# IRMVLab/EfficientLO-Net

Measured on AMD Instinct MI355X. Metric: frame-pairs/sec (KITTI 64x1800 range image), higher is better.
Workload: dtype f32 (1x1 convolutions as 3 fp16-MFMA products of hi/lo-split fp32 operands, fp32 accumulate)

## Files before the change

efficientlo-net_amd/_lib.py:

```python
import ctypes
import os

import torch

_PKG = os.path.dirname(os.path.abspath(__file__))
LIB_PATH = os.environ.get("ELO_LIB_PATH") or os.path.join(
    _PKG, "libelo_hip_f32.so" if os.environ.get("ELO_DENSE_F32", "0") == "1" else "libelo_hip.so")

_vp = ctypes.c_void_p


class GroupArgs(ctypes.Structure):
    _fields_ = [("batch", ctypes.c_int), ("H", ctypes.c_int), ("W", ctypes.c_int),
                ("H2", ctypes.c_int), ("W2", ctypes.c_int), ("npoints", ctypes.c_int),
                ("kernel_h", ctypes.c_int), ("kernel_w", ctypes.c_int), ("K", ctypes.c_int),
                ("flag_copy", ctypes.c_int), ("distance", ctypes.c_float),
                ("stride_h", ctypes.c_int), ("stride_w", ctypes.c_int),
                ("xyz1", _vp), ("xyz2", _vp), ("idx_n2", _vp), ("random_hw", _vp),
                ("selected_bhw_idx", _vp), ("valid_idx", _vp), ("valid_in_dis_idx", _vp),
                ("selected_mask", _vp)]


def _struct(name, fields):
    return type(name, (ctypes.Structure,), {"_fields_": fields, "__doc__": "struct %s (include/elo.h)." % name})


_i, _f = ctypes.c_int, ctypes.c_float
GroupConcatArgs = _struct("elo_group_concat_args", [
    ("batch", _i), ("npoints", _i), ("K", _i), ("H2", _i), ("W2", _i), ("C", _i),
    ("centre_xyz", _vp), ("src_xyz", _vp), ("src_feat", _vp), ("idx", _vp), ("mask", _vp), ("out", _vp)])
MaskedMaxpoolArgs = _struct("elo_masked_maxpool_args", [
    ("batch", _i), ("npoints", _i), ("K", _i), ("C", _i), ("x", _vp), ("mask", _vp), ("out", _vp)])
CvEncode1Args = _struct("elo_cv_encode1_args", [
    ("batch", _i), ("npoints", _i), ("K", _i), ("H2", _i), ("W2", _i), ("C", _i),
    ("xyz1", _vp), ("feat1", _vp), ("xyz2", _vp), ("feat2", _vp), ("idx", _vp), ("mask", _vp), ("out", _vp),
    ("dtype", _i)])
CvEncode2Args = _struct("elo_cv_encode2_args", [
    ("batch", _i), ("npoints", _i), ("K", _i), ("H", _i), ("W", _i), ("C", _i), ("Cc", _i),
    ("xyz1", _vp), ("feat1", _vp), ("cost", _vp), ("idx", _vp), ("mask", _vp), ("xyz_cat", _vp), ("rest", _vp),
    ("dtype", _i)])
SoftmaxPoolArgs = _struct("elo_softmax_pool_args", [
    ("batch", _i), ("npoints", _i), ("K", _i), ("C", _i), ("logits", _vp), ("values", _vp),
    ("values_stride", _i), ("mask", _vp), ("out", _vp), ("dtype", _i)])
ELO_F32, ELO_F16 = 0, 1
SoftmaxValidArgs = _struct("elo_softmax_valid_args", [
    ("batch", _i), ("npoints", _i), ("C", _i), ("feature", _vp), ("weight", _vp), ("xyz", _vp), ("out", _vp),
    ("scratch", _vp), ("stats", _vp)])
SV_MAX_PARTS = 512
PermRefreshArgs = _struct("elo_perm_refresh_args", [
    ("pool", _vp), ("versions", _i), ("total", _i), ("cursor", _vp), ("flat", _vp), ("decoded", _vp), ("entry_of", _vp),
    ("table", _vp), ("n_entries", _i)])
PoseHeadArgs = _struct("elo_pose_head_args", [
    ("batch", _i), ("npoints", _i), ("C", _i), ("hidden", _i), ("feature", _vp), ("weight", _vp), ("xyz", _vp),
    ("W_big", _vp), ("b_big", _vp), ("W_q", _vp), ("b_q", _vp), ("W_t", _vp), ("b_t", _vp),
    ("q_coarse", _vp), ("t_coarse", _vp), ("q", _vp), ("t", _vp), ("q_norm", _vp), ("scratch", _vp), ("pose7", _vp),
    ("clear_scratch", _vp), ("clear_xyz", _vp), ("clear_feat", _vp), ("clear_cells", ctypes.c_long), ("clear_C", _i),
    ("feat_dtype", _i), ("pose7_slots", _i), ("pose7_cursor", _vp), ("next_orders", PermRefreshArgs), ("ready_parts", _i)])
WarpProjectArgs = _struct("elo_warp_project_args", [
    ("batch", _i), ("npoints", _i), ("C", _i), ("H", _i), ("W", _i),
    ("az_res", _f), ("vert_res", _f), ("vert_off", _f),
    ("xyz", _vp), ("feat", _vp), ("q", _vp), ("t", _vp), ("warped", _vp), ("out_xyz", _vp), ("out_feat", _vp),
    ("scratch", _vp), ("prepared", _i), ("feat_dtype", _i)])

InputStageArgs = _struct("elo_input_stage_args", [
    ("batch", _i), ("npoints", _i), ("point_stride", _i), ("H", _i), ("W", _i), ("az_res", _f), ("vert_res", _f),
    ("vert_off", _f), ("crop_xy", _f), ("cloud", _vp), ("T_trans", _vp), ("aug_frame", _vp), ("points", _vp),
    ("out_xyz", _vp), ("scratch", _vp)])
PreprocessGtArgs = _struct("elo_preprocess_gt_args", [
    ("batch", _i), ("T_gt", _vp), ("T_trans", _vp), ("T_trans_inv", _vp), ("aug_frame", _vp), ("q_gt", _vp), ("t_gt", _vp)])

GroupConcatBwdArgs = _struct("elo_group_concat_bwd_args", [
    ("batch", _i), ("npoints", _i), ("K", _i), ("H2", _i), ("W2", _i), ("C", _i),
    ("grad_out", _vp), ("idx", _vp), ("mask", _vp), ("grad_centre", _vp), ("grad_src_xyz", _vp), ("grad_src_feat", _vp)])
MaskedMaxpoolBwdArgs = _struct("elo_masked_maxpool_bwd_args", [
    ("batch", _i), ("npoints", _i), ("K", _i), ("C", _i), ("x", _vp), ("mask", _vp), ("grad_out", _vp), ("grad_x", _vp)])
CvEncode1BwdArgs = _struct("elo_cv_encode1_bwd_args", [
    ("batch", _i), ("npoints", _i), ("K", _i), ("H2", _i), ("W2", _i), ("C", _i),
    ("xyz1", _vp), ("xyz2", _vp), ("idx", _vp), ("mask", _vp), ("grad_out", _vp),
    ("grad_xyz1", _vp), ("grad_feat1", _vp), ("grad_xyz2", _vp), ("grad_feat2", _vp)])
CvEncode2BwdArgs = _struct("elo_cv_encode2_bwd_args", [
    ("batch", _i), ("npoints", _i), ("K", _i), ("H", _i), ("W", _i), ("C", _i), ("Cc", _i),
    ("xyz1", _vp), ("idx", _vp), ("mask", _vp), ("grad_xyz_cat", _vp), ("grad_rest", _vp),
    ("grad_xyz1", _vp), ("grad_feat1", _vp), ("grad_cost", _vp)])
SoftmaxPoolBwdArgs = _struct("elo_softmax_pool_bwd_args", [
    ("batch", _i), ("npoints", _i), ("K", _i), ("C", _i), ("logits", _vp), ("values", _vp), ("values_stride", _i),
    ("mask", _vp), ("grad_out", _vp), ("grad_logits", _vp), ("grad_values", _vp)])
SoftmaxValidBwdArgs = _struct("elo_softmax_valid_bwd_args", [
    ("batch", _i), ("npoints", _i), ("C", _i), ("feature", _vp), ("weight", _vp), ("xyz", _vp), ("grad_out", _vp),
    ("grad_feature", _vp), ("grad_weight", _vp), ("out", _vp), ("stats", _vp)])
WarpProjectBwdArgs = _struct("elo_warp_project_bwd_args", [
    ("batch", _i), ("npoints", _i), ("C", _i), ("H", _i), ("W", _i), ("az_res", _f), ("vert_res", _f), ("vert_off", _f),
    ("xyz", _vp), ("q", _vp), ("t", _vp), ("scratch", _vp), ("grad_out_xyz", _vp), ("grad_out_feat", _vp),
    ("grad_warped", _vp), ("grad_xyz", _vp), ("grad_feat", _vp), ("grad_q", _vp), ("grad_t", _vp)])

BnStatsArgs = _struct("elo_bn_stats_args", [
    ("rows", ctypes.c_long), ("C", _i), ("z", _vp), ("scratch", _vp), ("eps", _f), ("momentum", _f), ("mean", _vp), ("invstd", _vp),
    ("running_mean", _vp), ("running_var", _vp), ("groups", _i)])
BnApplyArgs = _struct("elo_bn_apply_args", [
    ("rows", ctypes.c_long), ("C", _i), ("z", _vp), ("mean", _vp), ("invstd", _vp), ("gamma", _vp), ("beta", _vp), ("relu", _i),
    ("y", _vp), ("groups", _i)])
BnBackwardArgs = _struct("elo_bn_backward_args", [
    ("rows", ctypes.c_long), ("C", _i), ("dy", _vp), ("z", _vp), ("mean", _vp), ("invstd", _vp), ("gamma", _vp), ("beta", _vp),
    ("relu", _i), ("scratch", _vp), ("sums", _vp), ("dz", _vp), ("groups", _i)])
AdamFlatArgs = _struct("elo_adam_flat_args", [
    ("n", ctypes.c_long), ("param", _vp), ("grad", _vp), ("exp_avg", _vp), ("exp_avg_sq", _vp), ("hyper", _vp),
    ("beta1", _f), ("beta2", _f), ("one_minus_beta1", _f), ("one_minus_beta2", _f)])
PoseComposeArgs = _struct("elo_pose_compose_args", [
    ("batch", _i), ("q_raw", _vp), ("t_det", _vp), ("q_coarse", _vp), ("t_coarse", _vp), ("q", _vp), ("t", _vp), ("q_norm", _vp),
    ("grad_q", _vp), ("grad_t", _vp), ("grad_q_norm", _vp), ("grad_q_raw", _vp), ("grad_t_det", _vp), ("grad_q_coarse", _vp),
    ("grad_t_coarse", _vp)])
# ... 40 lines not shown
    ("setconv_chain_rows", _l), ("mlp_chain_rows", _l), ("small_tile_units", _l), ("pool_wave", _i)])

SYMBOLS = [
    ("elo_abi_version", ctypes.c_int, []),
    ("elo_dense_f32", ctypes.c_int, []),
    ("elo_last_error", ctypes.c_char_p, []),
    ("elo_range_check", ctypes.c_int, [ctypes.c_int]),
    ("elo_range_violations", ctypes.c_int, [ctypes.POINTER(ctypes.c_ulonglong), _vp]),
    ("elo_get_tuning", ctypes.c_int, [ctypes.POINTER(Tuning)]),
    ("elo_set_tuning", ctypes.c_int, [ctypes.POINTER(Tuning)]),
    ("elo_fused_conv_random_k", ctypes.c_int, [ctypes.POINTER(GroupArgs), _vp]),
    ("elo_fused_conv_select_k", ctypes.c_int, [ctypes.POINTER(GroupArgs), _vp]),
    ("elo_fused_conv_random_k_dense", ctypes.c_int, [ctypes.POINTER(GroupArgs), _vp]),
    ("elo_fused_conv_select_k_dense", ctypes.c_int, [ctypes.POINTER(GroupArgs), _vp]),
    ("elo_fused_conv_random_k_dense_fits", ctypes.c_int, [ctypes.c_int] * 5),
    ("elo_fused_conv_select_k_dense_fits", ctypes.c_int, [ctypes.c_int] * 6),
    ("elo_debug_select_dense_waves", ctypes.c_int, [ctypes.c_int]),
    ("elo_perm_refresh", ctypes.c_int, [ctypes.POINTER(PermRefreshArgs), _vp]),
    ("elo_group_concat", ctypes.c_int, [ctypes.POINTER(GroupConcatArgs), _vp]),
    ("elo_masked_maxpool", ctypes.c_int, [ctypes.POINTER(MaskedMaxpoolArgs), _vp]),
    ("elo_cv_encode1", ctypes.c_int, [ctypes.POINTER(CvEncode1Args), _vp]),
    ("elo_cv_encode2", ctypes.c_int, [ctypes.POINTER(CvEncode2Args), _vp]),
    ("elo_masked_softmax_pool", ctypes.c_int, [ctypes.POINTER(SoftmaxPoolArgs), _vp]),
    ("elo_softmax_valid", ctypes.c_int, [ctypes.POINTER(SoftmaxValidArgs), _vp]),
    ("elo_pose_head", ctypes.c_int, [ctypes.POINTER(PoseHeadArgs), _vp]),
    ("elo_warp_project", ctypes.c_int, [ctypes.POINTER(WarpProjectArgs), _vp]),
    ("elo_input_stage", ctypes.c_int, [ctypes.POINTER(InputStageArgs), _vp]),
    ("elo_preprocess_gt", ctypes.c_int, [ctypes.POINTER(PreprocessGtArgs), _vp]),
    ("elo_pose_head_warp", ctypes.c_int, [ctypes.POINTER(PoseHeadArgs), ctypes.POINTER(WarpProjectArgs), _vp]),
    ("elo_group_concat_backward", ctypes.c_int, [ctypes.POINTER(GroupConcatBwdArgs), _vp]),
    ("elo_masked_maxpool_backward", ctypes.c_int, [ctypes.POINTER(MaskedMaxpoolBwdArgs), _vp]),
    ("elo_cv_encode1_backward", ctypes.c_int, [ctypes.POINTER(CvEncode1BwdArgs), _vp]),
    ("elo_cv_encode2_backward", ctypes.c_int, [ctypes.POINTER(CvEncode2BwdArgs), _vp]),
    ("elo_masked_softmax_pool_backward", ctypes.c_int, [ctypes.POINTER(SoftmaxPoolBwdArgs), _vp]),
    ("elo_softmax_valid_backward", ctypes.c_int, [ctypes.POINTER(SoftmaxValidBwdArgs), _vp]),
    ("elo_warp_project_backward", ctypes.c_int, [ctypes.POINTER(WarpProjectBwdArgs), _vp]),
    ("elo_bn_stats", ctypes.c_int, [ctypes.POINTER(BnStatsArgs), _vp]),
    ("elo_bn_apply", ctypes.c_int, [ctypes.POINTER(BnApplyArgs), _vp]),
    ("elo_bn_backward", ctypes.c_int, [ctypes.POINTER(BnBackwardArgs), _vp]),
    ("elo_dense_weight_grad", ctypes.c_int, [ctypes.POINTER(WeightGradArgs), _vp]),
    ("elo_dense_rows", ctypes.c_int, [ctypes.POINTER(DenseRowsArgs), _vp]),
    ("elo_dense_rows_supported", ctypes.c_int, [ctypes.c_long, ctypes.c_int, ctypes.c_int]),
    ("elo_dense_rows_scratch_floats", ctypes.c_long, [ctypes.c_int, ctypes.c_int]),
    ("elo_bn_scratch_floats", ctypes.c_long, [ctypes.c_int, ctypes.c_int]),
    ("elo_adam_flat", ctypes.c_int, [ctypes.POINTER(AdamFlatArgs), _vp]),
    ("elo_pose_compose", ctypes.c_int, [ctypes.POINTER(PoseComposeArgs), _vp]),
    ("elo_pose_loss", ctypes.c_int, [ctypes.POINTER(PoseLossArgs), _vp]),
    ("elo_weight_grad_slices", ctypes.c_int, [ctypes.c_long, ctypes.c_int, ctypes.c_int]),
    ("elo_setconv_fused", ctypes.c_int, [ctypes.POINTER(SetconvArgs), _vp]),
    ("elo_mlp_fused", ctypes.c_int, [ctypes.POINTER(MlpArgs), _vp]),
    ("elo_setconv_fused2", ctypes.c_int, [ctypes.POINTER(SetconvArgs), ctypes.POINTER(SetconvArgs), _vp]),
    ("elo_mlp_fused2", ctypes.c_int, [ctypes.POINTER(MlpArgs), ctypes.POINTER(MlpArgs), _vp]),
    ("elo_mlp_sv_parts", ctypes.c_int, [ctypes.POINTER(MlpArgs), ctypes.POINTER(MlpArgs)]),
    ("elo_cv_stage1_fused", ctypes.c_int, [ctypes.POINTER(Cv1Args), _vp]),
    ("elo_debug_cv1_rr", ctypes.c_int, [ctypes.c_int]),
    ("elo_debug_rr_rows", ctypes.c_int, [ctypes.c_long, ctypes.c_long]),
    ("elo_debug_rr_launches", ctypes.c_int, [ctypes.POINTER(ctypes.c_ulonglong), ctypes.c_int]),
    ("elo_debug_narrow_mfma", ctypes.c_int, [ctypes.c_int]),
    ("elo_debug_narrow_launches", ctypes.c_int, [ctypes.POINTER(ctypes.c_ulonglong), ctypes.c_int]),
    ("elo_debug_sv_ride_launches", ctypes.c_int, [ctypes.POINTER(ctypes.c_ulonglong), ctypes.c_int]),
    ("elo_get_tuning_base", ctypes.c_int, [ctypes.POINTER(Tuning)]),
    ("elo_graph_submit", ctypes.c_int, [_vp, _vp, _vp, _vp, ctypes.c_ulong, _vp, _vp, ctypes.c_int]),
    ("elo_debug_chain_pair_launches", ctypes.c_int, [ctypes.POINTER(ctypes.c_ulonglong), ctypes.c_int]),
    ("elo_cv_stage1_setconv_chain_form", ctypes.c_int, [ctypes.POINTER(Cv1Args), ctypes.POINTER(SetconvArgs), ctypes.POINTER(SetconvArgs)]),
    ("elo_cv_stage1_setconv_chain", ctypes.c_int, [ctypes.POINTER(Cv1Args), ctypes.POINTER(SetconvArgs), ctypes.POINTER(SetconvArgs), _vp]),
    ("elo_cv_stage2_fused", ctypes.c_int, [ctypes.POINTER(Cv2Args), _vp]),
    ("elo_debug_upconv_ride_launches", ctypes.c_int, [ctypes.POINTER(ctypes.c_ulonglong), ctypes.c_int]),
    ("elo_cv_stage2_upconv_form", ctypes.c_int, [ctypes.POINTER(Cv2Args), ctypes.POINTER(MlpArgs), ctypes.POINTER(MlpArgs)]),
    ("elo_cv_stage2_upconv_fused", ctypes.c_int, [ctypes.POINTER(Cv2Args), ctypes.POINTER(MlpArgs), ctypes.POINTER(MlpArgs), _vp]),
    ("elo_cv_stage1_setconv_fused", ctypes.c_int, [ctypes.POINTER(Cv1Args), ctypes.POINTER(SetconvArgs), ctypes.POINTER(SetconvArgs), _vp]),
]

_lib = None


class EloError(RuntimeError):
    pass


ABI_VERSION = 26


def lib():
    global _lib
    if _lib is None:
        if not os.path.exists(LIB_PATH):
            raise EloError("libelo_hip.so is not built (%s); run `python -c 'import __graft_entry__ as g; "
                           "g.build()'` -- there is no CPU fallback for the hot path" % LIB_PATH)
        handle = ctypes.CDLL(LIB_PATH)
        for name, restype, argtypes in SYMBOLS:
            fn = getattr(handle, name)
            fn.restype = restype
            fn.argtypes = argtypes
        if handle.elo_abi_version() != ABI_VERSION:
            raise EloError("%s has ABI version %d, this host expects %d: rebuild (python -c 'import __graft_entry__ as g; "
                           "g.build()')" % (LIB_PATH, handle.elo_abi_version(), ABI_VERSION))
        _lib = handle
        from . import tuning
        env = tuning.lib_from_env()
        if env:
            set_tuning(**env)
    return _lib


def get_tuning():
    t = Tuning()
# ... 8 lines not shown


def set_tuning(**fields):
    t = Tuning()
    check(lib().elo_get_tuning_base(ctypes.byref(t)))
    for name, value in fields.items():
        if not hasattr(t, name):
            raise KeyError("elo_tuning has no field %r" % name)
        setattr(t, name, int(value))
    check(lib().elo_set_tuning(ctypes.byref(t)))
    from . import tuning
    tuning.bump()


def check(rc):
    if rc != 0:
        raise EloError("libelo_hip: %s (status %d)" % (lib().elo_last_error().decode(), rc))


_range_counter = None


def set_range_counter(ptr):
    global _range_counter
    prev, _range_counter = _range_counter, ptr
    return prev


def _stamp(*structs):
    if _range_counter is not None:
        for a in structs:
            if a is not None and hasattr(a, "range_counter"):
                a.range_counter = _range_counter


def call(entry, args, like):
    _stamp(args)
    with torch.cuda.device(like.device):
        check(getattr(lib(), entry)(ctypes.byref(args), stream_ptr(like)))


def call3(entry, a, b, c, like):
    _stamp(a, b, c)
    with torch.cuda.device(like.device):
        check(getattr(lib(), entry)(ctypes.byref(a), ctypes.byref(b), ctypes.byref(c) if c is not None else None, stream_ptr(like)))


def call2(entry, args_a, args_b, like):
    _stamp(args_a, args_b)
    with torch.cuda.device(like.device):
        check(getattr(lib(), entry)(ctypes.byref(args_a), ctypes.byref(args_b), stream_ptr(like)))


def call2n(entry, args_a, args_b, like):
    _stamp(args_a, args_b)
    with torch.cuda.device(like.device):
        check(getattr(lib(), entry)(ctypes.byref(args_a), ctypes.byref(args_b) if args_b is not None else None, stream_ptr(like)))


def stream_ptr(t):
    return ctypes.c_void_p(torch.cuda.current_stream(t.device).cuda_stream)


def require_gpu(*tensors):
    for t in tensors:
        if t is not None and not t.is_cuda:
            raise EloError("the EfficientLO-Net hot path runs on an AMD GPU only (got a %s tensor); "
                           "there is no CPU fallback" % t.device)


def dtype_code(t):
    if t.dtype == torch.float32:
        return ELO_F32
    if t.dtype == torch.float16:
        return ELO_F16
    raise TypeError("feature tensors are float32 or float16 (got %s)" % t.dtype)


def range_check(enable):
    return lib().elo_range_check(1 if enable else 0)


def range_violations(like):
    n = ctypes.c_ulonglong(0)
    with torch.cuda.device(like.device):
        check(lib().elo_range_violations(ctypes.byref(n), stream_ptr(like)))
    return int(n.value)
```

efficientlo-net_amd/_ops.py:

```python
import math

import numpy as np

import ctypes

import torch

from . import _lib as L
from . import tuning


def _wants_grad(*ts):
    return torch.is_grad_enabled() and any(t is not None and t.requires_grad for t in ts)


_ptr = lambda x: x.data_ptr() if x is not None else None


def _feature_dtype(*ts):
    dt = ts[0].dtype
    if dt not in (torch.float32, torch.float16) or any(t.dtype != dt for t in ts):
        raise TypeError("cost-volume feature tensors are all float32 or all float16 (got %s)" % [str(t.dtype) for t in ts])
    return [t.contiguous() for t in ts], dt, L.ELO_F16 if dt == torch.float16 else L.ELO_F32

# ... 293 lines not shown
    f = lambda x, n: None if x is None else _f32(x.reshape(B, n))[0]
    return _PoseCompose.apply(f(q_raw, 4), f(t_det, 3), f(q_coarse, 4), f(t_coarse, 3))


class _PoseLoss(torch.autograd.Function):

    @staticmethod
    def forward(ctx, w_x, w_q, q_gt, t_gt, *poses):
        B = q_gt.shape[0]
        loss = torch.empty((), dtype=torch.float32, device=q_gt.device)
        P4 = ctypes.c_void_p * 4
        a = L.PoseLossArgs(B, P4(*[poses[2 * i].data_ptr() for i in range(4)]), P4(*[poses[2 * i + 1].data_ptr() for i in range(4)]),
                           q_gt.data_ptr(), t_gt.data_ptr(), w_x.data_ptr(), w_q.data_ptr(), loss.data_ptr(), None, P4(), P4(), None, None)
        L.call("elo_pose_loss", a, q_gt)
        ctx.save_for_backward(w_x, w_q, q_gt, t_gt, *poses)
        return loss

    @staticmethod
    def backward(ctx, grad_out):
        w_x, w_q, q_gt, t_gt, *poses = ctx.saved_tensors
        B = q_gt.shape[0]
        grads = [torch.empty_like(x) for x in poses]
        g_wx, g_wq = torch.empty_like(w_x), torch.empty_like(w_q)
        go = grad_out.contiguous().float()
        P4 = ctypes.c_void_p * 4
        a = L.PoseLossArgs(B, P4(*[poses[2 * i].data_ptr() for i in range(4)]), P4(*[poses[2 * i + 1].data_ptr() for i in range(4)]),
                           q_gt.data_ptr(), t_gt.data_ptr(), w_x.data_ptr(), w_q.data_ptr(), None, go.data_ptr(),
                           P4(*[grads[2 * i].data_ptr() for i in range(4)]), P4(*[grads[2 * i + 1].data_ptr() for i in range(4)]),
                           g_wx.data_ptr(), g_wq.data_ptr())
        L.call("elo_pose_loss", a, q_gt)
        return (g_wx, g_wq, None, None) + tuple(grads)


def pose_loss(l0_q, l0_t, l1_q, l1_t, l2_q, l2_t, l3_q, l3_t, q_gt, t_gt, w_x, w_q):
    L.require_gpu(l0_q, q_gt, w_x)
    B = q_gt.shape[0]
    poses = [_f32(x.reshape(B, n))[0] for x, n in ((l0_q, 4), (l0_t, 3), (l1_q, 4), (l1_t, 3), (l2_q, 4), (l2_t, 3), (l3_q, 4), (l3_t, 3))]
    return _PoseLoss.apply(w_x, w_q, _f32(q_gt.reshape(B, 4))[0], _f32(t_gt.reshape(B, 3))[0], *poses)


class ProjectionBuffers:

    def __init__(self, B, N, H, W, C, device, dtype=torch.float32):
        self.shape = (B, N, H, W, C)
        self.out_xyz = torch.empty((B, H, W, 3), dtype=torch.float32, device=device)
        self.out_feat = torch.empty((B, H, W, C), dtype=dtype, device=device) if C else None
        self.scratch = torch.empty((B * H * W + 4 * B + 2 * B * N,), dtype=torch.int32, device=device)
        self.cleared = False
        self.result = None


class SvPartials:

    def __init__(self, xyz_bn3, feature_bnc=None):
        (self.xyz,) = _f32(xyz_bn3)
        self.feature = feature_bnc
        self.scratch = torch.empty((3 * xyz_bn3.shape[0] * L.SV_MAX_PARTS * 64,), dtype=torch.float32, device=xyz_bn3.device)
        self.parts = 0


class PoseRing:

    def __init__(self, slots, batch, device):
        if slots < 2:
            raise ValueError("a pose ring has at least 2 slots")
        self.rows = torch.zeros((slots, batch, 7), dtype=torch.float32, device=device)
        self.cursor = torch.zeros((batch,), dtype=torch.int32, device=device)
        self.slots = slots

    def reset(self):
        self.cursor.zero_()


def pose_head(feature_bnc, weight_bnc, xyz_bn3, W_big, b_big, W_q, b_q, W_t, b_t, q_coarse=None, t_coarse=None, pose7=None,
              clear=None, warp=None, next_orders=None, partials=None):
    L.require_gpu(feature_bnc, weight_bnc, xyz_bn3, W_big, W_q, W_t, q_coarse, t_coarse)
    xyz_bn3, W_big, b_big, W_q, b_q, W_t, b_t = _f32(xyz_bn3, W_big, b_big, W_q, b_q, W_t, b_t)
    (feature_bnc, weight_bnc), fdt, fcode = _feature_dtype(feature_bnc, weight_bnc)
    B, N, C = feature_bnc.shape
    hidden = W_big.shape[1]
    dev = feature_bnc.device
    if q_coarse is not None:
        q_coarse, t_coarse = _f32(q_coarse.reshape(B, 4), t_coarse.reshape(B, 3))
    q = torch.empty((B, 4), dtype=torch.float32, device=dev)
    t = torch.empty((B, 3), dtype=torch.float32, device=dev)
    q_norm = torch.empty((B, 4), dtype=torch.float32, device=dev)
    ready = partials.parts if partials is not None else 0
    if ready and C != 64:
        raise ValueError("partials= goes with the 64-channel head")
    scratch = partials.scratch if ready else torch.empty((3 * B * L.SV_MAX_PARTS * C,), dtype=torch.float32, device=dev)
    ptr = lambda x: x.data_ptr() if x is not None else None
    ring = pose7 if isinstance(pose7, PoseRing) else None
    if ring is not None:
        if ring.rows.shape[1] != B:
            raise ValueError("pose ring of batch %d used with batch %d" % (ring.rows.shape[1], B))
        pose7 = ring.rows
    a = L.PoseHeadArgs(B, N, C, hidden, feature_bnc.data_ptr(), weight_bnc.data_ptr(), xyz_bn3.data_ptr(),
                       W_big.data_ptr(), b_big.data_ptr(), W_q.data_ptr(), b_q.data_ptr(), W_t.data_ptr(), b_t.data_ptr(),
                       ptr(q_coarse), ptr(t_coarse), q.data_ptr(), t.data_ptr(), q_norm.data_ptr(), scratch.data_ptr(),
                       ptr(pose7), *((clear.scratch.data_ptr(), clear.out_xyz.data_ptr(), ptr(clear.out_feat),
                                      clear.shape[0] * clear.shape[2] * clear.shape[3], clear.shape[4])
                                     if clear is not None else (None, None, None, 0, 0)), fcode,
                       ring.slots if ring is not None else 0, ring.cursor.data_ptr() if ring is not None else None,
                       next_orders if next_orders is not None else L.PermRefreshArgs(), ready)
    if ready and clear is not None and not clear.cleared:
        raise ValueError("partials=: the ProjectionBuffers must have been cleared by an earlier launch (fused.mlp(clear=...))")
    if clear is not None and clear.out_feat is not None and clear.out_feat.dtype != fdt:
        raise TypeError("the projection buffers and the pose head's features must share one storage dtype")
    if warp is not None:
        if clear is None:
            raise ValueError("warp= needs clear= (the ProjectionBuffers the projection writes)")
        xyz_w, feat_w = warp
        (xyz_w,) = _f32(xyz_w)
        Bw, Nw, Hw, Ww, Cw = clear.shape
        if xyz_w.shape != (Bw, Nw, 3) or (Cw and (feat_w is None or feat_w.shape != (Bw, Nw, Cw))):
            raise ValueError("warp inputs do not match the ProjectionBuffers %s" % (clear.shape,))
        if feat_w is not None:
            if feat_w.dtype != fdt:
                raise TypeError("the warped features and the pose head's features must share one storage dtype")
            feat_w = feat_w.contiguous()
        warped = torch.empty((Bw, Nw, 3), dtype=torch.float32, device=dev)
        az, vres, voff = projection_constants(Hw, Ww)
        w = L.WarpProjectArgs(Bw, Nw, Cw, Hw, Ww, az, vres, voff, xyz_w.data_ptr(), ptr(feat_w), None, None,
                              warped.data_ptr(), clear.out_xyz.data_ptr(), ptr(clear.out_feat), clear.scratch.data_ptr(), 1, fcode)
        L.call2("elo_pose_head_warp", a, w, q)
        clear.result = (warped, clear.out_xyz, clear.out_feat)
        return q, t, q_norm
    L.call("elo_pose_head", a, q)
    if clear is not None:
        clear.cleared = True
    return q, t, q_norm


def projection_constants(H_input, W_input):
    d2r = math.pi / 180
    az = (360.0 / W_input) * d2r
    down, up = -24.8 * d2r, 2.0 * d2r
    vres = (up - down) / (H_input - 1)
    return az, vres, -down / vres


def _aug_frame_dev(aug_frame, B, dev):
    if isinstance(aug_frame, torch.Tensor) and aug_frame.dtype == torch.int32 and aug_frame.device == dev:
        if aug_frame.numel() != B or not aug_frame.is_contiguous():
            raise ValueError("a device aug_frame is a contiguous int32 tensor of one entry per batch element")
        return aug_frame.view(B)
    return torch.as_tensor(np.asarray(aug_frame).reshape(B), dtype=torch.int32).to(dev)


def preprocess_gt(T_gt, T_trans, T_trans_inv, aug_frame_dev):
    L.require_gpu(T_gt, T_trans, T_trans_inv)
    B = T_gt.shape[0]
    (T_gt,) = _f32(T_gt.reshape(B, 4, 4))
    dev = T_gt.device
    if (T_trans is None) != (T_trans_inv is None):
        raise ValueError("T_trans and T_trans_inv come together")
    aug = None
    if T_trans is not None:
        T_trans, T_trans_inv = _f32(T_trans.reshape(B, 4, 4), T_trans_inv.reshape(B, 4, 4))
        if not isinstance(aug_frame_dev, torch.Tensor) or aug_frame_dev.dtype != torch.int32:
            raise TypeError("aug_frame_dev is an int32 tensor on the device (the launch reads it there)")
        L.require_gpu(aug_frame_dev)
        aug = _aug_frame_dev(aug_frame_dev, B, dev)
    q_gt = torch.empty((B, 4), dtype=torch.float32, device=dev)
    t_gt = torch.empty((B, 3), dtype=torch.float32, device=dev)
    a = L.PreprocessGtArgs(B, T_gt.data_ptr(), _ptr(T_trans), _ptr(T_trans_inv), _ptr(aug), q_gt.data_ptr(), t_gt.data_ptr())
    L.call("elo_preprocess_gt", a, q_gt)
    return q_gt, t_gt


def input_stage(cloud, T_trans, aug_frame, H, W, crop_xy=35.0):
    L.require_gpu(cloud, T_trans)
    (cloud,) = _f32(cloud)
    B, N2, S = cloud.shape
    if N2 % 2 or S < 3:
        raise ValueError("point_cloud must be (B, 2*N, >=3)")
    N, dev = N2 // 2, cloud.device
    if T_trans is not None:
        (T_trans,) = _f32(T_trans.reshape(B, 4, 4))
        aug = _aug_frame_dev(aug_frame, B, dev)
    points = torch.empty((2 * B, N, 3), dtype=torch.float32, device=dev)
# ... 191 lines not shown
```

efficientlo-net_amd/csrc/elo_features.hip:

```cpp
#include <type_traits>
#include "elo_common.h"
#include "elo_project_device.h"

namespace elo {
namespace {

constexpr int ROWS_PER_BLOCK = ELO_BLOCK / ELO_WAVE;

__device__ __forceinline__ long row_of_wave(long total_rows)
{
    const long r = (long)xcd_tile(blockIdx.x, gridDim.x) * ROWS_PER_BLOCK + threadIdx.x / ELO_WAVE;
    return r < total_rows ? r : -1;
}

inline unsigned grid_for_rows(long rows) { return (unsigned)((rows + ROWS_PER_BLOCK - 1) / ROWS_PER_BLOCK); }

constexpr int STAGE_ROWS = 64;

__device__ __forceinline__ void stream_out(const float *tile, float *__restrict__ dst, long first_row, long rows, int CT)
{
    const long valid = (rows - first_row < STAGE_ROWS ? rows - first_row : STAGE_ROWS) * CT;
    float *o = dst + first_row * CT;
    const long vec = valid >> 2;
    for (long i = threadIdx.x; i < vec; i += ELO_BLOCK)
        reinterpret_cast<float4 *>(o)[i] = reinterpret_cast<const float4 *>(tile)[i];
    for (long i = (vec << 2) + threadIdx.x; i < valid; i += ELO_BLOCK) o[i] = tile[i];
}

inline unsigned grid_for_stage(long rows) { return (unsigned)((rows + STAGE_ROWS - 1) / STAGE_ROWS); }

struct StageMeta { long *cell; float *mask; };

__device__ __forceinline__ StageMeta stage_meta(float *after_tile, long first, long rows, const int *__restrict__ idx,
                                                const float *__restrict__ mask, int H2, int W2)
{
    StageMeta m{reinterpret_cast<long *>(after_tile), after_tile + 2 * STAGE_ROWS};
    const int t = threadIdx.x;
    if (t < STAGE_ROWS) {
        const long r = first + t;
        long cell = -1;
        float mk = 0.0f;
        if (r < rows) {
            const int *id = idx + r * 3;
            cell = ((long)id[0] * H2 + id[1]) * W2 + id[2];
            mk = mask[r];
        }
        m.cell[t] = cell;
        m.mask[t] = mk;
    }
    __syncthreads();
    return m;
}

constexpr size_t STAGE_META_BYTES = sizeof(float) * 3 * STAGE_ROWS;

// ... 487 lines not shown
    auto add2 = [](float x, float y) { return x + y; };
#pragma unroll
    for (int c = 0; c < E; ++c) mx[c] = across_groups<LPR>(mx[c], fmax2);
    float den[E], acc[E];
#pragma unroll
    for (int c = 0; c < E; ++c) den[c] = acc[c] = 0.0f;
#pragma unroll
    for (int j = 0; j < J; ++j)
#pragma unroll
        for (int c = 0; c < E; ++c) {
            const float e = live[j] ? ex(lv[j][c] - mx[c]) : 0.0f;
            den[c] += e;
            acc[c] += e * (float)v4[j][c];
        }
#pragma unroll
    for (int c = 0; c < E; ++c) {
        den[c] = across_groups<LPR>(den[c], add2);
        acc[c] = across_groups<LPR>(acc[c], add2);
    }
    if (g == 0 && mine) {
        V16 o;
#pragma unroll
        for (int c = 0; c < E; ++c) o[c] = (T)(acc[c] / den[c]);
        STREAM_STORE(o, &reinterpret_cast<V16 *>(static_cast<T *>(a.out) + r * 64)[sub]);
    }
}

__global__ __launch_bounds__(ELO_BLOCK) void softmax_pool_kernel(const elo_softmax_pool_args a, const long rows)
{
    const long r = row_of_wave(rows);
    if (r < 0) return;
    const int lane = threadIdx.x % ELO_WAVE;
    const float *lg = static_cast<const float *>(a.logits) + r * a.K * a.C;
    const float *vl = static_cast<const float *>(a.values) + r * a.K * (long)a.values_stride;
    const float *m = a.mask + r * a.K;
    float *outp = static_cast<float *>(a.out);
    for (int c = lane; c < a.C; c += ELO_WAVE) {
        float mx = -INFINITY;
        for (int k = 0; k < a.K; ++k) {
            const float l = m[k] == 1.0f ? lg[(long)k * a.C + c] : -1e10f;
            mx = fmaxf(mx, l);
        }
        float den = 0.0f, acc = 0.0f;
        for (int k = 0; k < a.K; ++k) {
            const float l = m[k] == 1.0f ? lg[(long)k * a.C + c] : -1e10f;
            const float e = expf(l - mx);
            den += e;
            acc += e * vl[(long)k * a.values_stride + c];
        }
        outp[r * a.C + c] = acc / den;
    }
}

struct SvPartials {
    float *mx, *den, *acc;
};

__device__ __forceinline__ SvPartials sv_partials(float *scratch, int batch, int C)
{
    const size_t n = (size_t)batch * ELO_SV_MAX_PARTS * C;
    return SvPartials{scratch, scratch + n, scratch + 2 * n};
}

template <bool F16>
__global__ __launch_bounds__(ELO_BLOCK) void softmax_valid_partial_kernel(const void *__restrict__ feature_,
                                                                          const void *__restrict__ weight_,
                                                                          const float *__restrict__ xyz, int npoints,
                                                                          int C, int parts, float *scratch,
                                                                          const ProjectionClear clear)
{
    typedef typename std::conditional<F16, _Float16, float>::type feat_t;
    const feat_t *__restrict__ feature = reinterpret_cast<const feat_t *>(feature_);
    const feat_t *__restrict__ weight = reinterpret_cast<const feat_t *>(weight_);
    auto ex = [](float x) { return exp_acc(x); };
    __shared__ float part[3][ROWS_PER_BLOCK][ELO_WAVE];
    clear_projection(clear);
    const int slice = blockIdx.x, b = blockIdx.y, lane = threadIdx.x % ELO_WAVE, wave = threadIdx.x / ELO_WAVE;
    const int c = blockIdx.z * ELO_WAVE + lane;
    const bool live = c < C;
    const int cc = live ? c : C - 1;
    const long fbase = (long)b * npoints * C;
    const float *p = xyz + (long)b * npoints * 3;
    const int per = (npoints + parts - 1) / parts;
    const int lo = slice * per, hi = min(npoints, lo + per);
    float mx = -INFINITY, den = 0.0f, acc = 0.0f;
    constexpr int SV_ROWS = 16;
    for (int n0 = lo + wave; n0 < hi; n0 += SV_ROWS * ROWS_PER_BLOCK) {
        float l[SV_ROWS], v[SV_ROWS];
        bool ok[SV_ROWS];
#pragma unroll
        for (int u = 0; u < SV_ROWS; ++u) {
            const int n = n0 + u * ROWS_PER_BLOCK;
            const int nn = n < hi ? n : hi - 1;
            const float px = p[nn * 3 + 0], py = p[nn * 3 + 1], pz = p[nn * 3 + 2];
            l[u] = (float)weight[fbase + (long)nn * C + cc];
            v[u] = (float)feature[fbase + (long)nn * C + cc];
            ok[u] = (n < hi) & live & !((px == 0.0f) & (py == 0.0f) & (pz == 0.0f));
        }
        float bm = -INFINITY;
#pragma unroll
        for (int u = 0; u < SV_ROWS; ++u) bm = ok[u] ? fmaxf(bm, l[u]) : bm;
        if (bm > -INFINITY) {
            float d16 = 0.0f, a16 = 0.0f;
#pragma unroll
            for (int u = 0; u < SV_ROWS; ++u) {
                const float e = ok[u] ? ex(l[u] - bm) : 0.0f;
                d16 += e;
                a16 += e * v[u];
            }
            const float m2 = fmaxf(mx, bm), s0 = ex(mx - m2), s1 = ex(bm - m2);
            den = den * s0 + d16 * s1;
            acc = acc * s0 + a16 * s1;
            mx = m2;
        }
    }
    part[0][wave][lane] = mx; part[1][wave][lane] = den; part[2][wave][lane] = acc;
    __syncthreads();
    if (wave == 0 && live) {
        float M = -INFINITY;
        for (int i = 0; i < ROWS_PER_BLOCK; ++i) M = fmaxf(M, part[0][i][lane]);
        float D = 0.0f, A = 0.0f;
        for (int i = 0; i < ROWS_PER_BLOCK; ++i) {
            if (part[1][i][lane] == 0.0f) continue;
            const float sc = ex(part[0][i][lane] - M);
            D += part[1][i][lane] * sc;
            A += part[2][i][lane] * sc;
        }
        const SvPartials o = sv_partials(scratch, gridDim.y, C);
        const size_t at = ((size_t)b * ELO_SV_MAX_PARTS + slice) * C + c;
        o.mx[at] = M; o.den[at] = D; o.acc[at] = A;
    }
}

__device__ __forceinline__ float sv_merge(const SvPartials &s, int b, int c, int C, int parts)
{
    float M = -INFINITY;
    for (int i = 0; i < parts; ++i) M = fmaxf(M, s.mx[((size_t)b * ELO_SV_MAX_PARTS + i) * C + c]);
    float D = 0.0f, A = 0.0f;
    for (int i = 0; i < parts; ++i) {
        const size_t at = ((size_t)b * ELO_SV_MAX_PARTS + i) * C + c;
        if (s.den[at] == 0.0f) continue;
        const float sc = expf(s.mx[at] - M);
        D += s.den[at] * sc;
        A += s.acc[at] * sc;
    }
    return D > 0.0f ? A / D : 0.0f;
}

__global__ void softmax_valid_merge_kernel(float *scratch, int batch, int C, int parts, float *out, float *stats)
{
    const int i = blockIdx.x * blockDim.x + threadIdx.x;
    if (i >= batch * C) return;
    const SvPartials s = sv_partials(scratch, batch, C);
    const int b = i / C, c = i % C;
    out[i] = sv_merge(s, b, c, C, parts);
    if (stats) {
        float M = -INFINITY, D = 0.0f;
        for (int k = 0; k < parts; ++k) M = fmaxf(M, s.mx[((size_t)b * ELO_SV_MAX_PARTS + k) * C + c]);
        for (int k = 0; k < parts; ++k) {
            const size_t at = ((size_t)b * ELO_SV_MAX_PARTS + k) * C + c;
            if (s.den[at] != 0.0f) D += s.den[at] * expf(s.mx[at] - M);
        }
        stats[((size_t)b * 2) * C + c] = M;
        stats[((size_t)b * 2 + 1) * C + c] = D;
    }
}

struct ProjScratch { unsigned *minr, *zflag; int *cell_of; unsigned *rbits; };

__host__ __device__ inline ProjScratch proj_scratch(unsigned *s, size_t cells, size_t images, size_t pts)
{
    return ProjScratch{s, s + cells, (int *)(s + cells + ZFLAGS * images), s + cells + ZFLAGS * images + pts};
}

__device__ __forceinline__ void bin_point(float x, float y, float z, long i, int b, int H, int W, float az_res, float vert_res,
                                          float vert_off, const ProjScratch &ps)
{
    const float r = sqrtf(x * x + y * y + z * z);
    const float at = atan2f(y, x);
    const int cell = cell_of_point(at, z, r, H, W, az_res, vert_res, vert_off);
    const unsigned rb = __float_as_uint(r);
    ps.cell_of[i] = cell;
    ps.rbits[i] = rb;
    if (rb == 0) {
        const int flag = b * ZFLAGS + zero_kind(at);
        const unsigned long long zeros = __ballot(1);
        const int leader = __ffsll((long long)zeros) - 1;
        if ((int)(threadIdx.x & 63) == leader || flag != __shfl(flag, leader)) ps.zflag[flag] = 0u;
        return;
    }
    unsigned *slot = ps.minr + (long)b * H * W + cell;
    if (__hip_atomic_load(slot, __ATOMIC_RELAXED, __HIP_MEMORY_SCOPE_AGENT) > rb) atomicMin(slot, rb);
}

__device__ __forceinline__ void warp_cell_point(const elo_warp_project_args &a, long i, int b, const float *q, const float *t,
                                                const ProjScratch &ps)
{
    float x = a.xyz[i * 3 + 0], y = a.xyz[i * 3 + 1], z = a.xyz[i * 3 + 2];
    if (q) {
        const bool keep = !(x == 0.0f && y == 0.0f && z == 0.0f);
        const float q0 = q[0], q1 = q[1], q2 = q[2], q3 = q[3];
        const float v0 = q0 * 0.0f - q1 * x - q2 * y - q3 * z;
        const float v1 = q0 * x + q1 * 0.0f + q2 * z - q3 * y;
        const float v2 = q0 * y - q1 * z + q2 * 0.0f + q3 * x;
        const float v3 = q0 * z + q1 * y - q2 * x + q3 * 0.0f;
        const float n2 = q0 * q0 + q1 * q1 + q2 * q2 + q3 * q3 + 1e-10f;
        const float i0 = q0 / n2, i1 = -q1 / n2, i2 = -q2 / n2, i3 = -q3 / n2;
        const float w1 = v0 * i1 + v1 * i0 + v2 * i3 - v3 * i2;
        const float w2 = v0 * i2 - v1 * i3 + v2 * i0 + v3 * i1;
        const float w3 = v0 * i3 + v1 * i2 - v2 * i1 + v3 * i0;
        const float k = keep ? 1.0f : 0.0f;
        x = (w1 + t[0]) * k; y = (w2 + t[1]) * k; z = (w3 + t[2]) * k;
        a.warped[i * 3 + 0] = x; a.warped[i * 3 + 1] = y; a.warped[i * 3 + 2] = z;
    }
    bin_point(x, y, z, i, b, a.H, a.W, a.az_res, a.vert_res, a.vert_off, ps);
}

__device__ __forceinline__ void hamilton(const float *a, const float *b, float *r)
{
    r[0] = a[0] * b[0] - a[1] * b[1] - a[2] * b[2] - a[3] * b[3];
    r[1] = a[0] * b[1] + a[1] * b[0] + a[2] * b[3] - a[3] * b[2];
    r[2] = a[0] * b[2] - a[1] * b[3] + a[2] * b[0] + a[3] * b[1];
    r[3] = a[0] * b[3] + a[1] * b[2] - a[2] * b[1] + a[3] * b[0];
}

__device__ __forceinline__ void normalise_q(const float *q, float *o)
{
    const float n = sqrtf(q[0] * q[0] + q[1] * q[1] + q[2] * q[2] + q[3] * q[3] + 1e-10f) + 1e-10f;
    for (int i = 0; i < 4; ++i) o[i] = q[i] / n;
}

#ifdef ELO_POSE_CLOCK
__device__ unsigned long long g_pose_clock[4 * 8 + 1];
#define POSE_STAMP(i) do { if (blockIdx.x == 0 && blockIdx.y == 0 && threadIdx.x == 0) {                                    \
        if ((i) == 0) pose_slot = (int)(g_pose_clock[32]++ % 4);                                                          \
        g_pose_clock[pose_slot * 8 + (i)] = __builtin_readcyclecounter(); } } while (0)
#else
#define POSE_STAMP(i) do { } while (0)
#endif

template <int BLOCK>
__global__ __launch_bounds__(BLOCK) void pose_head_kernel(const elo_pose_head_args a, const int parts,
                                                          const elo_warp_project_args w, const int with_warp)
{
    extern __shared__ float sm[];
    float *feat = sm, *big = sm + a.C, *head = big + a.hidden;
    const int b = blockIdx.y, tid = threadIdx.x;
    const SvPartials s = sv_partials(a.scratch, gridDim.y, a.C);
#ifdef ELO_POSE_CLOCK
    int pose_slot = 0;
#endif
    POSE_STAMP(0);
    constexpr int HEAD_C = 64;
    const bool model_head = a.C == HEAD_C && a.hidden == BLOCK;
    float wb[HEAD_C], wq[4], wt[3], bias_big = 0.0f;
    auto request_weights = [&]() {
        const int j = tid;
#pragma unroll
        for (int c = 0; c < HEAD_C; ++c) wb[c] = a.W_big[(size_t)c * a.hidden + j];
#pragma unroll
        for (int o = 0; o < 4; ++o) wq[o] = a.W_q[(size_t)j * 4 + o];
#pragma unroll
        for (int o = 0; o < 3; ++o) wt[o] = a.W_t[(size_t)j * 3 + o];
        bias_big = a.b_big[j];
    };
    float *mpart = head + 8 + 8 * (BLOCK / ELO_WAVE);
    if (model_head) request_weights();
    const int c = tid & 63, q = tid >> 6;
    float M = -INFINITY, D = 0.0f, A = 0.0f;
    if (c < a.C) {
        auto trips = [&](auto mine) {
            constexpr int MINE = decltype(mine)::value;
            for (int i0 = q; i0 < parts; i0 += 4 * MINE) {
                float m_[MINE], d_[MINE], a_[MINE];
#pragma unroll
                for (int u = 0; u < MINE; ++u) {
                    const int i = i0 + 4 * u;
                    const size_t at = ((size_t)b * ELO_SV_MAX_PARTS + (i < parts ? i : 0)) * a.C + c;
                    m_[u] = s.mx[at]; a_[u] = s.acc[at];
                    d_[u] = i < parts ? s.den[at] : 0.0f;
                }
#pragma unroll
                for (int u = 0; u < MINE; ++u) {
                    if (d_[u] == 0.0f) continue;
                    if (m_[u] > M) { const float sc = exp_acc(M - m_[u]); D = D * sc + d_[u]; A = A * sc + a_[u]; M = m_[u]; }
                    else { const float sc = exp_acc(m_[u] - M); D += d_[u] * sc; A += a_[u] * sc; }
                }
            }
        };
        if (parts <= 64) trips(std::integral_constant<int, 16>());
        else trips(std::integral_constant<int, 32>());
    }
    POSE_STAMP(1);
    mpart[(0 * 4 + q) * 64 + c] = M; mpart[(1 * 4 + q) * 64 + c] = D; mpart[(2 * 4 + q) * 64 + c] = A;
    __syncthreads();
    if (tid < 64) {
        float MM = -INFINITY;
        for (int i = 0; i < 4; ++i) MM = fmaxf(MM, mpart[(0 * 4 + i) * 64 + tid]);
        float DD = 0.0f, AA = 0.0f;
        for (int i = 0; i < 4; ++i) {
            if (mpart[(1 * 4 + i) * 64 + tid] == 0.0f) continue;
            const float sc = exp_acc(mpart[(0 * 4 + i) * 64 + tid] - MM);
            DD += mpart[(1 * 4 + i) * 64 + tid] * sc; AA += mpart[(2 * 4 + i) * 64 + tid] * sc;
        }
        if (tid < a.C) feat[tid] = DD > 0.0f ? AA / DD : 0.0f;
    }
    for (int c2 = 64 + tid; c2 < a.C; c2 += blockDim.x) feat[c2] = sv_merge(s, b, c2, a.C, parts);

    __syncthreads();
    POSE_STAMP(2);
    if (model_head) {
        float v = bias_big;
#pragma unroll
        for (int c = 0; c < HEAD_C; ++c) v += feat[c] * wb[c];
        big[tid] = v;
    } else {
        for (int j = tid; j < a.hidden; j += blockDim.x) {
            float v = a.b_big[j];
#pragma unroll 16
            for (int c = 0; c < a.C; ++c) v += feat[c] * a.W_big[(size_t)c * a.hidden + j];
            big[j] = v;
        }
    }
    __syncthreads();
    POSE_STAMP(3);
    {
        float part[7] = {0, 0, 0, 0, 0, 0, 0};
        if (model_head) {
            const float bj = big[tid];
#pragma unroll
            for (int o = 0; o < 4; ++o) part[o] += bj * wq[o];
#pragma unroll
            for (int o = 0; o < 3; ++o) part[4 + o] += bj * wt[o];
        } else {
            for (int j = tid; j < a.hidden; j += blockDim.x) {
                const float bj = big[j];
#pragma unroll
                for (int o = 0; o < 4; ++o) part[o] += bj * a.W_q[(size_t)j * 4 + o];
#pragma unroll
                for (int o = 0; o < 3; ++o) part[4 + o] += bj * a.W_t[(size_t)j * 3 + o];
            }
        }
#pragma unroll
        for (int o = 0; o < 7; ++o)
            for (int d = 32; d >= 1; d >>= 1) part[o] += __shfl_xor(part[o], d, ELO_WAVE);
        float *wsum = head + 8;
        if ((tid & 63) == 0)
            for (int o = 0; o < 7; ++o) wsum[(tid >> 6) * 8 + o] = part[o];
        __syncthreads();
        if (tid < 7) {
            float v = tid < 4 ? a.b_q[tid] : a.b_t[tid - 4];
            for (int w = 0; w < (int)(blockDim.x >> 6); ++w) v += wsum[w * 8 + tid];
            head[tid] = v;
        }
    }
    __syncthreads();
    POSE_STAMP(4);
    if (tid == 0) {
        float q_det[4], q[4], t[3], qn[4];
        normalise_q(head, q_det);
        const float *t_det = head + 4;
        if (a.q_coarse) {
            const float *qc = a.q_coarse + b * 4, *tc = a.t_coarse + b * 3;
            const float tq[4] = {0.0f, tc[0], tc[1], tc[2]};
            float v[4], w[4], inv[4];
            hamilton(q_det, tq, v);
            const float n2 = q_det[0] * q_det[0] + q_det[1] * q_det[1] + q_det[2] * q_det[2] + q_det[3] * q_det[3] + 1e-10f;
            inv[0] = q_det[0] / n2; inv[1] = -q_det[1] / n2; inv[2] = -q_det[2] / n2; inv[3] = -q_det[3] / n2;
            hamilton(v, inv, w);
            hamilton(q_det, qc, q);
            for (int i = 0; i < 3; ++i) t[i] = w[i + 1] + t_det[i];
        } else {
            for (int i = 0; i < 4; ++i) q[i] = q_det[i];
            for (int i = 0; i < 3; ++i) t[i] = t_det[i];
        }
        normalise_q(q, qn);
        if (blockIdx.x == 0) {
            for (int i = 0; i < 4; ++i) { a.q[b * 4 + i] = q[i]; a.q_norm[b * 4 + i] = qn[i]; }
            for (int i = 0; i < 3; ++i) a.t[b * 3 + i] = t[i];
            if (a.pose7) {
                float *row = a.pose7 + b * 7;
                if (a.pose7_slots > 1 && a.pose7_cursor) {
                    const unsigned at = a.pose7_cursor[b];
                    a.pose7_cursor[b] = at + 1u;
                    row += (size_t)(at % (unsigned)a.pose7_slots) * a.batch * 7;
                }
                for (int i = 0; i < 4; ++i) row[i] = qn[i];
                for (int i = 0; i < 3; ++i) row[4 + i] = t[i];
            }
        }
        if (with_warp) {
            for (int i = 0; i < 4; ++i) head[8 + i] = q[i];
            for (int i = 0; i < 3; ++i) head[12 + i] = t[i];
        }
    }
    POSE_STAMP(5);
    if (a.next_orders.pool && blockIdx.x == 0 && blockIdx.y == 0) perm_refresh_block(a.next_orders);
    POSE_STAMP(6);
    if (!with_warp) return;
    __syncthreads();
    const long n = (long)blockIdx.x * blockDim.x + tid;
    if (n < w.npoints) {
        warp_cell_point(w, (long)b * w.npoints + n, b, head + 8, head + 12,
                        proj_scratch(w.scratch, (size_t)w.batch * w.H * w.W, w.batch, (size_t)w.batch * w.npoints));
    }
    POSE_STAMP(7);
}

__global__ __launch_bounds__(ELO_BLOCK) void project_init_kernel(unsigned *minr, float *out_xyz, unsigned *out_feat,
                                                                 size_t cells, int C, int images)
{
    const size_t n_xyz = cells * 3, n_feat = cells * (size_t)C, total = cells + n_xyz + n_feat;
    for (size_t i = (size_t)blockIdx.x * blockDim.x + threadIdx.x; i < (size_t)images * ZFLAGS; i += (size_t)gridDim.x * blockDim.x)
        minr[cells + i] = 0x7f7f7f7fu;
    for (size_t i = (size_t)blockIdx.x * blockDim.x + threadIdx.x; i < total; i += (size_t)gridDim.x * blockDim.x) {
        if (i < cells) minr[i] = 0x7f7f7f7fu;
        else if (i < cells + n_xyz) out_xyz[i - cells] = 0.0f;
        else out_feat[i - cells - n_xyz] = 0u;
    }
}

__global__ __launch_bounds__(ELO_BLOCK) void warp_cell_kernel(const elo_warp_project_args a, const ProjScratch ps)
{
    const long total = (long)a.batch * a.npoints;
    for (long i = (long)blockIdx.x * blockDim.x + threadIdx.x; i < total; i += (long)gridDim.x * blockDim.x) {
        const int b = point_batch(i, a.npoints);
        warp_cell_point(a, i, b, a.q ? a.q + b * 4 : nullptr, a.q ? a.t + b * 3 : nullptr, ps);
    }
}

__global__ __launch_bounds__(ELO_BLOCK) void input_cell_kernel(const elo_input_stage_args a, const ProjScratch ps)
{
    const long per_frame = (long)a.batch * a.npoints, total = 2 * per_frame;
    for (long i = (long)blockIdx.x * blockDim.x + threadIdx.x; i < total; i += (long)gridDim.x * blockDim.x) {
        const int f = i >= per_frame;
        const long j = i - f * per_frame;
        const int b = point_batch(j, a.npoints);
        const long n = j - (long)b * a.npoints;
        const float *p = a.cloud + ((long)b * 2 * a.npoints + (long)f * a.npoints + n) * a.point_stride;
        float x = p[0], y = p[1], z = p[2], w = 1.0f;
        const float valid = (x != 0.0f || y != 0.0f || z != 0.0f) ? 1.0f : 0.0f;
        if (sqrtf(__fadd_rn(__fmul_rn(x, x), __fmul_rn(y, y))) > a.crop_xy) x = y = z = w = 0.0f;
        if (a.T_trans && a.aug_frame[b] == f + 1) {
            const float *T = a.T_trans + b * 16;
            const float nx = T[0] * x + T[1] * y + T[2] * z + T[3] * w;
            const float ny = T[4] * x + T[5] * y + T[6] * z + T[7] * w;
            const float nz = T[8] * x + T[9] * y + T[10] * z + T[11] * w;
            x = nx; y = ny; z = nz;
        }
        x *= valid; y *= valid; z *= valid;
        a.points[i * 3 + 0] = x; a.points[i * 3 + 1] = y; a.points[i * 3 + 2] = z;
        bin_point(x, y, z, i, f * a.batch + b, a.H, a.W, a.az_res, a.vert_res, a.vert_off, ps);
    }
}

__global__ __launch_bounds__(64) void preprocess_gt_kernel(const elo_preprocess_gt_args a)
{
    const int b = blockIdx.x * blockDim.x + threadIdx.x;
    if (b >= a.batch) return;
// ... 232 lines not shown
            else hipLaunchKernelGGL((softmax_pool_vec_kernel<float, 6>), grid, dim3(ELO_BLOCK), 0, s, *a, rows);
        } else {
            if (a->dtype == ELO_F16) hipLaunchKernelGGL((softmax_pool_vec_kernel<half_t, 4, true>), grid, dim3(ELO_BLOCK), 0, s, *a, rows);
            else hipLaunchKernelGGL((softmax_pool_vec_kernel<float, 4>), grid, dim3(ELO_BLOCK), 0, s, *a, rows);
        }
        return check_launch(who);
    }
    hipLaunchKernelGGL(softmax_pool_kernel, dim3(grid_for_rows(rows)), dim3(ELO_BLOCK), 0, (hipStream_t)stream, *a, rows);
    return check_launch(who);
}

#ifdef ELO_POSE_CLOCK
extern "C" int elo_debug_pose_clock(unsigned long long *out33)
{
    return hipMemcpyFromSymbol(out33, HIP_SYMBOL(g_pose_clock), 33 * sizeof(unsigned long long)) == hipSuccess ? 0 : -3;
}
#endif

static int sv_parts(int npoints)
{
    constexpr int SV_MAX_SLICES = 64;
    int parts = (npoints + 63) / 64;
    return parts < 1 ? 1 : parts > SV_MAX_SLICES ? SV_MAX_SLICES : parts;
}

extern "C" int elo_softmax_valid(const elo_softmax_valid_args *a, elo_stream_t stream)
{
    const char *who = "elo_softmax_valid";
    ELO_REQUIRE(a, who, "null argument block");
    ELO_REQUIRE(a->batch >= 0 && a->npoints > 0 && a->C > 0, who, "bad sizes");
    ELO_REQUIRE(a->feature && a->weight && a->xyz && a->out && a->scratch, who, "null tensor pointer");
    if (a->batch == 0) return ELO_OK;
    const int parts = sv_parts(a->npoints);
    hipLaunchKernelGGL(softmax_valid_partial_kernel<false>, dim3(parts, a->batch, (a->C + ELO_WAVE - 1) / ELO_WAVE),
                       dim3(ELO_BLOCK), 0, (hipStream_t)stream, a->feature, a->weight, a->xyz, a->npoints, a->C, parts,
                       a->scratch, ProjectionClear{nullptr, nullptr, nullptr, 0, 0, 0});
    hipLaunchKernelGGL(softmax_valid_merge_kernel, dim3((a->batch * a->C + ELO_BLOCK - 1) / ELO_BLOCK), dim3(ELO_BLOCK),
                       0, (hipStream_t)stream, a->scratch, a->batch, a->C, parts, a->out, a->stats);
    return check_launch(who);
}

static int check_warp_project(const elo_warp_project_args *a, const char *who)
{
    ELO_REQUIRE(a, who, "null argument block");
    ELO_REQUIRE(a->batch >= 0 && a->npoints > 0 && a->C >= 0 && a->H > 0 && a->W > 0, who, "bad sizes");
    ELO_REQUIRE(a->xyz && a->out_xyz && a->scratch, who, "null tensor pointer");
    ELO_REQUIRE(a->C == 0 || (a->feat && a->out_feat), who, "features requested without buffers");
    ELO_REQUIRE(!a->q || (a->t && a->warped), who, "warp requested without t / warped");
    ELO_REQUIRE(a->feat_dtype == ELO_F32 || a->feat_dtype == ELO_F16, who, "feat_dtype must be ELO_F32 or ELO_F16");
    ELO_REQUIRE(a->feat_dtype == ELO_F32 || a->C % 2 == 0, who, "fp16 feature storage needs an even C");
    return ELO_OK;
}

static int pose_head_impl(const elo_pose_head_args *a, const elo_warp_project_args *w, elo_stream_t stream, const char *who)
{
    ELO_REQUIRE(a, who, "null argument block");
    ELO_REQUIRE(a->batch >= 0 && a->npoints > 0 && a->C > 0 && a->hidden > 0, who, "bad sizes");
    ELO_REQUIRE(a->feature && a->weight && a->xyz && a->W_big && a->b_big && a->W_q && a->b_q && a->W_t && a->b_t &&
                a->q && a->t && a->q_norm && a->scratch, who, "null tensor pointer");
    ELO_REQUIRE((a->q_coarse == nullptr) == (a->t_coarse == nullptr), who, "q_coarse and t_coarse go together");
    ELO_REQUIRE(!a->clear_scratch || (a->clear_xyz && a->clear_cells > 0 && a->clear_C >= 0 && (a->clear_feat || a->clear_C == 0)),
                who, "incomplete clear_* side job");
    ELO_REQUIRE(!a->clear_scratch || a->clear_cells * (a->clear_C > 3 ? a->clear_C : 3) < (1l << 31), who, "clear_* side job: more than 2^31 words");
    ELO_REQUIRE(a->feat_dtype == ELO_F32 || a->feat_dtype == ELO_F16, who, "feat_dtype must be ELO_F32 or ELO_F16");
    const int f16 = a->feat_dtype == ELO_F16;
    ELO_REQUIRE(!f16 || a->clear_C % 2 == 0, who, "fp16 feature storage needs an even clear_C");
    elo_warp_project_args wv{};
    if (w) {
        if (int rc = check_warp_project(w, who)) return rc;
        ELO_REQUIRE(w->batch == a->batch && w->warped, who, "the warp must have the pose head's batch and a `warped` output");
        ELO_REQUIRE(w->feat_dtype == a->feat_dtype, who, "the warp and the pose head must share one feat_dtype");
        ELO_REQUIRE(a->clear_scratch == w->scratch && a->clear_xyz == w->out_xyz && a->clear_feat == w->out_feat &&
                    a->clear_cells == (long)w->batch * w->H * w->W && a->clear_C == w->C, who,
                    "the warp's buffers must be the ones this call clears (clear_*)");
        wv = *w;
        wv.q = a->q;
        wv.t = a->t;
    }
    ELO_REQUIRE(a->ready_parts >= 0 && a->ready_parts <= ELO_SV_MAX_PARTS, who, "ready_parts is 0..ELO_SV_MAX_PARTS");
    ELO_REQUIRE(!a->ready_parts || a->C == 64, who, "ready_parts: the partial sums of an MLP launch are 64 channels wide");
    if (a->batch == 0) return ELO_OK;
    hipStream_t s = (hipStream_t)stream;
    {
        const int parts = a->ready_parts ? a->ready_parts : sv_parts(a->npoints);
        const ProjectionClear clear{a->clear_scratch, a->clear_xyz, (unsigned *)a->clear_feat, a->clear_cells,
                                    f16 ? a->clear_C / 2 : a->clear_C, a->batch};
        const dim3 pgrid(parts, a->batch, (a->C + ELO_WAVE - 1) / ELO_WAVE);
        if (a->ready_parts) {}
        else if (f16)
            hipLaunchKernelGGL(softmax_valid_partial_kernel<true>, pgrid, dim3(ELO_BLOCK), 0, s, a->feature, a->weight, a->xyz,
                               a->npoints, a->C, parts, a->scratch, clear);
        else
            hipLaunchKernelGGL(softmax_valid_partial_kernel<false>, pgrid, dim3(ELO_BLOCK), 0, s, a->feature, a->weight, a->xyz,
                               a->npoints, a->C, parts, a->scratch, clear);
        const size_t lds = sizeof(float) * ((size_t)a->C + a->hidden + 8 + 8 * (ELO_BLOCK / ELO_WAVE) + 3 * 4 * 64);
        const unsigned xb = w ? (unsigned)((w->npoints + ELO_BLOCK - 1) / ELO_BLOCK) : 1u;
        hipLaunchKernelGGL((pose_head_kernel<ELO_BLOCK>), dim3(xb, a->batch), dim3(ELO_BLOCK), lds, s, *a, parts, wv, w ? 1 : 0);
    }
    if (w) {
        const size_t cells = (size_t)w->batch * w->H * w->W, pts = (size_t)w->batch * w->npoints;
        const size_t elems = pts * (3 + (f16 ? w->C / 2 : w->C));
        const unsigned gb = (unsigned)((elems + ELO_BLOCK - 1) / ELO_BLOCK);
        hipLaunchKernelGGL(scatter_min_kernel, dim3(gb > 4096 ? 4096 : gb), dim3(ELO_BLOCK), 0, s, wv,
                           proj_scratch(w->scratch, cells, w->batch, pts));
    }
    return check_launch(who);
}

extern "C" int elo_pose_head(const elo_pose_head_args *a, elo_stream_t stream)
{
    return pose_head_impl(a, nullptr, stream, "elo_pose_head");
}

extern "C" int elo_pose_head_warp(const elo_pose_head_args *a, const elo_warp_project_args *w, elo_stream_t stream)
{
    const char *who = "elo_pose_head_warp";
    ELO_REQUIRE(w, who, "null warp block");
    return pose_head_impl(a, w, stream, who);
}

extern "C" int elo_input_stage(const elo_input_stage_args *a, elo_stream_t stream)
{
    const char *who = "elo_input_stage";
    ELO_REQUIRE(a, who, "null argument block");
    ELO_REQUIRE(a->batch >= 0 && a->npoints > 0 && a->H > 0 && a->W > 0 && a->point_stride >= 3, who, "bad sizes");
    ELO_REQUIRE((a->T_trans == nullptr) == (a->aug_frame == nullptr), who, "T_trans and aug_frame come together");
    ELO_REQUIRE(a->az_res > 0.0f && a->vert_res > 0.0f, who, "bad projection constants");
    if (a->batch == 0) return ELO_OK;
    ELO_REQUIRE(a->cloud && a->points && a->out_xyz && a->scratch, who, "null tensor pointer");
    hipStream_t s = (hipStream_t)stream;
    const size_t images = 2 * (size_t)a->batch, cells = images * a->H * a->W, pts = images * a->npoints;
    const ProjScratch ps = proj_scratch(a->scratch, cells, images, pts);
    const unsigned gi = (unsigned)((cells * 4 + ELO_BLOCK - 1) / ELO_BLOCK);
    hipLaunchKernelGGL(project_init_kernel, dim3(gi > 4096 ? 4096 : gi), dim3(ELO_BLOCK), 0, s, ps.minr, a->out_xyz,
                       (unsigned *)nullptr, cells, 0, (int)images);
    const unsigned ga = (unsigned)((pts + ELO_BLOCK - 1) / ELO_BLOCK);
    hipLaunchKernelGGL(input_cell_kernel, dim3(ga > 8192 ? 8192 : ga), dim3(ELO_BLOCK), 0, s, *a, ps);
    elo_warp_project_args w = {};
    w.batch = (int)images; w.npoints = a->npoints; w.C = 0; w.H = a->H; w.W = a->W;
    w.az_res = a->az_res; w.vert_res = a->vert_res; w.vert_off = a->vert_off;
    w.xyz = a->points; w.out_xyz = a->out_xyz; w.scratch = a->scratch;
    const size_t elems = pts * 3;
    const unsigned gb = (unsigned)((elems + ELO_BLOCK - 1) / ELO_BLOCK);
    hipLaunchKernelGGL(scatter_min_kernel, dim3(gb > 8192 ? 8192 : gb), dim3(ELO_BLOCK), 0, s, w, ps);
    return check_launch(who);
}

extern "C" int elo_preprocess_gt(const elo_preprocess_gt_args *a, elo_stream_t stream)
{
    const char *who = "elo_preprocess_gt";
    ELO_REQUIRE(a, who, "null argument block");
    ELO_REQUIRE(a->batch >= 0, who, "bad sizes");
    ELO_REQUIRE((a->T_trans == nullptr) == (a->T_trans_inv == nullptr) && (a->T_trans == nullptr) == (a->aug_frame == nullptr), who,
                "T_trans, T_trans_inv and aug_frame come together");
    if (a->batch == 0) return ELO_OK;
    ELO_REQUIRE(a->T_gt && a->q_gt && a->t_gt, who, "null tensor pointer");
    hipLaunchKernelGGL(preprocess_gt_kernel, dim3((unsigned)((a->batch + 63) / 64)), dim3(64), 0, (hipStream_t)stream, *a);
    return check_launch(who);
}

extern "C" int elo_warp_project(const elo_warp_project_args *a, elo_stream_t stream)
{
    const char *who = "elo_warp_project";
    if (int rc = check_warp_project(a, who)) return rc;
// ... 19 lines not shown
```

efficientlo-net_amd/csrc/elo_fused.hip:

```cpp
#include "elo_group_device.h"
#include "elo_project_device.h"
#include <atomic>
#include <cstdlib>
#include <type_traits>

namespace elo {
namespace {

typedef float f32x4 __attribute__((ext_vector_type(4)));
typedef _Float16 half4 __attribute__((ext_vector_type(4)));
typedef _Float16 half2v __attribute__((ext_vector_type(2)));

constexpr int FUSED_BLOCK = 256;
constexpr int FUSED_WAVES = 4;
__device__ __forceinline__ int ftid() { return (int)(threadIdx.x & (FUSED_BLOCK - 1)); }

constexpr int MODE_SPLIT = 0;
constexpr int MODE_HALF = 1;
constexpr int MODE_CHECKED = 2;

__device__ unsigned long long g_range_violations;
__device__ unsigned long long g_range_snapshot;
__global__ void range_take_kernel() { g_range_snapshot = atomicExch(&g_range_violations, 0ull); }

#ifdef ELO_CV1_CLOCK
#define CV1_STAMP(i) do { if (block == 0 && threadIdx.x == 0) g_cv1_clock[i] = __builtin_readcyclecounter(); } while (0)
#ifndef ELO_RR_CLOCK_BLOCK
#define ELO_RR_CLOCK_BLOCK 0
#endif
#define RR_STAMP(i) do { if (blockIdx.x == ELO_RR_CLOCK_BLOCK && (threadIdx.x & 63) == 0 && (threadIdx.x >> 6) % 7 == 0) \
                             g_cv1_clock[(i) + 12 * (threadIdx.x >> 9 | (threadIdx.x >> 6) / 7)] = __builtin_readcyclecounter(); } while (0)
#ifdef ELO_RR_CLOCK_POOL
#define RR_POOL_STAMP(i) RR_STAMP(i)
#define RR_LAYER_STAMP(i) do { } while (0)
#else
#define RR_POOL_STAMP(i) do { } while (0)
#define RR_LAYER_STAMP(i) RR_STAMP(i)
#endif
#else
#define CV1_STAMP(i) do { } while (0)
#define RR_STAMP(i) do { } while (0)
#define RR_POOL_STAMP(i) do { } while (0)
#define RR_LAYER_STAMP(i) do { } while (0)
#endif

__device__ __forceinline__ int ceil8(int x) { return (x + 7) & ~7; }
__device__ __forceinline__ int ceil16(int x) { return (x + 15) & ~15; }

__host__ __device__ __forceinline__ int row_stride(int cols)
{
    int s = (cols + 3) & ~3;
    for (;; s += 4) {
        const int m = s & 63;
        if (m == 4 || m == 8 || m == 24 || m == 40 || m == 56) return s;
// ... 999 lines not shown
            }
            act_put<MODE>(act, row * S + ch, v, bad);
        }
    }
    __syncthreads();
    const int N = a.layers[a.n_layers - 1].N;
    const bool two = a.n_layers2 > 0;
    for (int l = 0; l < a.n_layers; ++l)
        dense<TILE, MODE>(act, S, 0, a.layers[l],
                          l == a.n_layers - 1 ? LayerOut{two || keep_final ? 0 : -1, !two && keep_final ? 1 : 0, a.out, first, end, f16} : to_tile(0), bad);
    if (!two) return;
    const int wb = a.w_before, wa = a.w_after, CT2 = N + wb + wa;
    if ((N & 3) == 0 && (wb == 0 || seg_ok(a.before, wb, TILE, f16)) && (wa == 0 || seg_ok(a.after, wa, TILE, f16))) {
        uint4 rb[SEG_ITEMS], ra[SEG_ITEMS];
        if (wb) seg_load<TILE>(rb, a.before, wb, f16, row_of);
        if (wa) seg_load<TILE>(ra, a.after, wa, f16, row_of);
        if (wb) seg_store<TILE, MODE>(act, S, N, wb, f16, rb, row_of, all, bad);
        if (wa) seg_store<TILE, MODE>(act, S, N + wb, wa, f16, ra, row_of, all, bad);
    } else {
        for (int e = tid; e < TILE * (wb + wa); e += FUSED_BLOCK) {
            const int row = small_div(e, wb + wa), ch = e - row * (wb + wa);
            const long gr = first + row;
            const long grc = gr < end ? gr : end - 1;
            const float v = ch < wb ? feat_load(a.before, grc * wb + ch, f16) : feat_load(a.after, grc * wa + (ch - wb), f16);
            act_put<MODE>(act, row * S + N + ch, gr < end ? v : 0.0f, bad);
        }
    }
    zero_cols<TILE, MODE>(act, S, CT2, ceil16(CT2));
    __syncthreads();
    for (int l = 0; l < a.n_layers2; ++l)
        dense<TILE, MODE>(act, S, 0, a.layers2[l],
                          l == a.n_layers2 - 1 ? LayerOut{keep_final ? 0 : -1, keep_final ? 1 : 0, a.out2, first, end, f16} : to_tile(0), bad);
}

template <int TILE, int MODE>
__global__ __launch_bounds__(FUSED_BLOCK, TILE == 32 ? ELO_TILE32_WAVES : ELO_TILE_WAVES) void mlp_kernel(const JobPair<elo_mlp_args> jobs, const int S)
{
    const elo_mlp_args &a = jobs.job[blockIdx.y];
    extern __shared__ __align__(16) float lds[];
    unsigned bad = 0;
    {
        const elo_mlp_args &j0 = jobs.job[0];
        clear_projection(ProjectionClear{j0.clear_scratch, j0.clear_xyz, (unsigned *)j0.clear_feat, j0.clear_cells,
                                         j0.feat_dtype == ELO_F16 ? j0.clear_C / 2 : j0.clear_C, j0.clear_images});
    }
    const long first = (long)xcd_tile(blockIdx.x, gridDim.x) * TILE;
    if (first >= a.rows) return;
    mlp_tile<TILE, MODE>(a, lds, S, first, a.rows, false, bad);
    report_violations<MODE>(bad, a.range_counter);
}

template <int TILE, int MODE, bool PAIR>
__global__ __launch_bounds__(PAIR ? 2 * FUSED_BLOCK : FUSED_BLOCK, TILE == 32 ? 4 : ELO_TILE_WAVES)
void mlp_sv_kernel(const JobPair<elo_mlp_args> jobs, const int S, const int tiles_pb)
{
    constexpr int C = 64;
    const int group = PAIR ? __builtin_amdgcn_readfirstlane(threadIdx.x >> 8) : 0;
    const elo_mlp_args &j0 = jobs.job[0];
    const elo_mlp_args &a = jobs.job[group];
    extern __shared__ __align__(16) float lds[];
    const int tile_words = TILE * S;
    float *act = lds + group * tile_words;
    float *staged = lds + (PAIR ? 2 : 1) * tile_words;
    unsigned bad = 0;
    clear_projection(ProjectionClear{j0.clear_scratch, j0.clear_xyz, (unsigned *)j0.clear_feat, j0.clear_cells,
                                     j0.feat_dtype == ELO_F16 ? j0.clear_C / 2 : j0.clear_C, j0.clear_images});
    const unsigned tile = xcd_tile(blockIdx.x, gridDim.x);
    const int b = (int)(tile / (unsigned)tiles_pb), t = (int)(tile - (unsigned)b * (unsigned)tiles_pb);
    const long first = (long)b * j0.sv_npoints + (long)t * TILE, end = (long)(b + 1) * j0.sv_npoints;
    const int f16 = j0.feat_dtype == ELO_F16;
    const int vr = threadIdx.x < TILE ? (int)threadIdx.x : 0;
    const long vrow = first + vr < end ? first + vr : end - 1;
    const float px = j0.sv_xyz[vrow * 3 + 0], py = j0.sv_xyz[vrow * 3 + 1], pz = j0.sv_xyz[vrow * 3 + 2];
    constexpr int STAGE = PAIR ? 1 : TILE / 16;
    uint4 held[STAGE];
    if constexpr (!PAIR) {
#pragma unroll
        for (int u = 0; u < STAGE; ++u) {
            const int e = (int)threadIdx.x + u * FUSED_BLOCK, fr = e >> 4, q = e & 15;
            const long grow = first + fr < end ? first + fr : end - 1;
            if (f16) { const uint2 h = reinterpret_cast<const uint2 *>(j0.sv_feature)[grow * (C / 4) + q]; held[u] = uint4{h.x, h.y, 0u, 0u}; }
            else held[u] = reinterpret_cast<const uint4 *>(j0.sv_feature)[grow * (C / 4) + q];
        }
    }
    mlp_tile<TILE, MODE>(a, act, S, first, end, true, bad);
    report_violations<MODE>(bad, a.range_counter);
    if constexpr (!PAIR) {
#pragma unroll
        for (int u = 0; u < STAGE; ++u) {
            const int e = (int)threadIdx.x + u * FUSED_BLOCK, fr = e >> 4, q = e & 15;
            float4 v;
            if (f16) {
                const half2v h0 = __builtin_bit_cast(half2v, held[u].x), h1 = __builtin_bit_cast(half2v, held[u].y);
                v = float4{(float)h0.x, (float)h0.y, (float)h1.x, (float)h1.y};
            } else {
                v = __builtin_bit_cast(float4, held[u]);
            }
            *reinterpret_cast<float4 *>(staged + fr * C + 4 * q) = v;
        }
        __syncthreads();
    }
    if (threadIdx.x >= C) return;
    const unsigned long long okm = __ballot((threadIdx.x < TILE) & (first + vr < end) & !((px == 0.0f) & (py == 0.0f) & (pz == 0.0f)));
    const int c = threadIdx.x;
    const float *logit = lds + c, *value = PAIR ? lds + tile_words + c : staged + c;
    const int vs = PAIR ? S : C;
    float M = -INFINITY, D = 0.0f, A = 0.0f;
#pragma unroll
    for (int r0 = 0; r0 < TILE; r0 += 16) {
        float l[16], v[16];
#pragma unroll
        for (int r = 0; r < 16; ++r) { l[r] = logit[(r0 + r) * S]; v[r] = value[(r0 + r) * vs]; }
        const unsigned ok = (unsigned)(okm >> r0) & 0xffffu;
        float bm = -INFINITY;
#pragma unroll
        for (int r = 0; r < 16; ++r) bm = (ok >> r & 1u) ? fmaxf(bm, l[r]) : bm;
        if (bm > -INFINITY) {
            float d16 = 0.0f, a16 = 0.0f;
#pragma unroll
            for (int r = 0; r < 16; ++r) {
                const float e = (ok >> r & 1u) ? exp_acc(l[r] - bm) : 0.0f;
                d16 += e;
                a16 += e * v[r];
            }
            const float m2 = fmaxf(M, bm), s0 = exp_acc(M - m2), s1 = exp_acc(bm - m2);
            D = D * s0 + d16 * s1;
            A = A * s0 + a16 * s1;
            M = m2;
        }
    }
    float *sc = j0.sv_scratch;
    const size_t n = (size_t)(gridDim.x / (unsigned)tiles_pb) * ELO_SV_MAX_PARTS * C;
    const size_t at = ((size_t)b * ELO_SV_MAX_PARTS + t) * C + c;
    sc[at] = M; sc[n + at] = D; sc[2 * n + at] = A;
}

__host__ __device__ __forceinline__ int cv1_feat_cols(int C)
{
    const int kp = (10 + 2 * C + 15) & ~15;
    return kp > 2 * C + 16 ? kp : 2 * C + 16;
}

__device__ __forceinline__ elo_dense kernarg_dense(size_t byte_offset)
{
    static_assert(sizeof(elo_dense) == 48, "three 16-byte scalar loads");
    typedef const __attribute__((address_space(4))) char *KernargBytes;
    typedef unsigned int Quad __attribute__((ext_vector_type(4)));
    typedef const __attribute__((address_space(4))) Quad *KernargQuads;
    KernargBytes p = (KernargBytes)__builtin_amdgcn_kernarg_segment_ptr() + byte_offset;
    asm volatile("" : "+s"(p));
    KernargQuads q = reinterpret_cast<KernargQuads>(p);
    struct Raw { Quad a, b, c; } raw = {q[0], q[1], q[2]};
    return __builtin_bit_cast(elo_dense, raw);
}
#define CV1_LAYER(field) kernarg_dense(offsetof(elo_cv1_args, field))

template <int TILE, int MODE, bool GROUP = true>
__device__ __forceinline__ void cv1_tile(const elo_cv1_args &a, const int S, float *lds, unsigned block, unsigned nblocks)
{
    float *act = lds;
    const TileMeta meta = tile_meta(lds, TILE, S);
    const int tid = threadIdx.x;
    const int K = a.K, P = TILE / K, C = a.C, f16 = a.feat_dtype == ELO_F16;
    unsigned bad = 0;
    const long total_points = (long)a.batch * a.npoints;
    const long first_point = (long)xcd_tile(block, nblocks) * P;
    if (first_point >= total_points) return;
    CV1_STAMP(0);
    if (GROUP && a.group.random_hw) {
        int *lds_off = reinterpret_cast<int *>(act);
        unsigned *scratch = reinterpret_cast<unsigned *>(lds_off + ((a.group.kernel_h * a.group.kernel_w + 3) & ~3));
        group_tile<TILE, true>(meta, lds_off, scratch, a.group, first_point, total_points, a.npoints, P, K, a.xyz1, a.H2,
                               a.W2, nullptr, a.xyz2, a.H2, a.W2, nullptr);
    } else {
        load_meta<TILE>(meta, first_point, total_points, P, K, a.idx, a.mask, a.H2, a.W2);
        __syncthreads();
    }
    CV1_STAMP(1);
    const int F = 128, G = F + 2 * C;
    {
        auto cell_of = [&](int row) { return (long)meta.cell[row]; };
        auto centre_of = [&](int row) { return meta.cell[row] >= 0 ? first_point + small_div(row, K) : -1L; };
        uint4 r1[SEG_ITEMS], r2[SEG_ITEMS];
        seg_load<TILE>(r1, a.feat1, C, f16, centre_of);
        seg_load<TILE>(r2, a.feat2, C, f16, cell_of);
        GeoRow gr;
        const bool grow = tid < TILE;
// ... 1364 lines not shown
{
    const int prev = tuning().chain_forms;
    tuning().chain_forms = on >= 0 ? (on != 0) : tuning_base().chain_forms;
    return prev;
}
static bool cv1_rr_on() { return tuning().chain_forms != 0; }
extern "C" int elo_debug_rr_rows(long setconv_rows, long mlp_rows)
{
    tuning().setconv_chain_rows = setconv_rows >= 0 ? setconv_rows : tuning_base().setconv_chain_rows;
    tuning().mlp_chain_rows = mlp_rows >= 0 ? mlp_rows : tuning_base().mlp_chain_rows;
    return ELO_OK;
}
static long setconv_rr_rows(int batch)
{
    const long t = tuning().setconv_chain_rows;
    (void)batch;
    return t >= 0 ? t : 20000L;
}
static long mlp_rr_rows(int batch_hint)
{
    const long t = tuning().mlp_chain_rows;
    return t >= 0 ? t : batch_hint >= ELO_THROUGHPUT_BATCH ? 2048L : 8192L;
}
extern "C" int elo_debug_narrow_mfma(int on)
{
    const int prev = tuning().narrow_mfma;
    tuning().narrow_mfma = on >= 0 ? (on ? 1 : 0) : tuning_base().narrow_mfma;
    return prev;
}
static bool narrow_mfma_on() { return tuning().narrow_mfma != 0; }
static std::atomic<unsigned long long> g_rr_launches[4];
extern "C" int elo_debug_rr_launches(unsigned long long *counts4, int reset)
{
    for (int i = 0; i < 4; ++i) {
        if (counts4) counts4[i] = g_rr_launches[i].load();
        if (reset) g_rr_launches[i].store(0);
    }
    return ELO_OK;
}
static std::atomic<unsigned long long> g_chain_pair_launches;
extern "C" int elo_debug_chain_pair_launches(unsigned long long *count, int reset)
{
    if (count) *count = g_chain_pair_launches.load();
    if (reset) g_chain_pair_launches.store(0);
    return ELO_OK;
}
static std::atomic<unsigned long long> g_upconv_ride_launches;
extern "C" int elo_debug_upconv_ride_launches(unsigned long long *count, int reset)
{
    if (count) *count = g_upconv_ride_launches.load();
    if (reset) g_upconv_ride_launches.store(0);
    return ELO_OK;
}
static std::atomic<unsigned long long> g_sv_ride_launches;
extern "C" int elo_debug_sv_ride_launches(unsigned long long *count, int reset)
{
    if (count) *count = g_sv_ride_launches.load();
    if (reset) g_sv_ride_launches.store(0);
    return ELO_OK;
}
static std::atomic<unsigned long long> g_narrow_launches[2];
extern "C" int elo_debug_narrow_launches(unsigned long long *counts2, int reset)
{
    for (int i = 0; i < 2; ++i) {
        if (counts2) counts2[i] = g_narrow_launches[i].load();
        if (reset) g_narrow_launches[i].store(0);
    }
    return ELO_OK;
}

static bool narrow_chain(const elo_setconv_args *a, const elo_setconv_args *b)
{
    return !b && a->K == 32 && a->n_layers == 3 && a->layers[0].w_plain && a->layers[1].w_plain && a->layers[2].w_plain;
}

static int setconv_chain_shape(const elo_setconv_args *a, const elo_setconv_args *b, int mode)
{
#ifdef ELO_DENSE_F32
    return 0;
#else
    const long points = (long)a->batch * a->npoints;
    const int nl = a->n_layers, n1 = a->layers[0].N, n2 = nl >= 2 ? a->layers[1].N : 0, n3 = nl == 3 ? a->layers[2].N : 0;
    const int shape = (nl == 2 && n1 == 128 && n2 == 64) ? 1 : (nl == 3 && n1 == 64 && n2 == 64 && n3 == 128) ? 2
                    : (nl == 3 && n1 == 128 && n2 == 64 && n3 == 64) ? 3 : 0;
    const int KT = a->group.kernel_h * a->group.kernel_w;
    if (!shape || narrow_chain(a, b) || !a->group.random_hw || !(mode == MODE_SPLIT || mode == MODE_HALF) || !cv1_rr_on() || a->C != 64 ||
        !(a->K == 8 || a->K == 16 || a->K == 32) || KT > 512 || a->group.idx_out || a->group.mask_out ||
        points * a->K * (b ? 2 : 1) < setconv_rr_rows(a->batch))
        return 0;
    return shape;
#endif
}

static bool cv_chain(int C, int mode)
{
#ifdef ELO_DENSE_F32
    return false;
#else
    return (mode == MODE_SPLIT || mode == MODE_HALF) && cv1_rr_on() && (C == 16 || C == 32 || C == 64);
#endif
}

extern "C" int elo_setconv_fused2(const elo_setconv_args *a, const elo_setconv_args *b, elo_stream_t stream)
{
    const char *who = "elo_setconv_fused";
    if (int rc = check_setconv(a, who)) return rc;
// ... 134 lines not shown
        for (int l = 0; same && l < a->n_layers; ++l) same = a->layers[l].N == b->layers[l].N;
        for (int l = 0; same && l < a->n_layers2; ++l) same = a->layers2[l].N == b->layers2[l].N;
        if (!same) return fail(ELO_ERR_ARG, "%s: the two jobs of a paired launch must have the same shape", who);
    }
    if (b && b->clear_scratch) return fail(ELO_ERR_ARG, "%s: the clear_* side job belongs to the first job of a pair", who);
    if (b && (b->sv_scratch || b->sv_feature)) return fail(ELO_ERR_ARG, "%s: the sv_* fields belong to the first job of a pair", who);
    p->S = row_stride(mlp_cols(a, in_width));
    const long u32 = (a->rows + 31) / 32;
    p->mode = 0;
    if (int rc = pair_products_mode(who, &p->mode, a->n_layers, a->n_layers2, a->layers, a->layers2, b ? b->layers : nullptr,
                                    b ? b->layers2 : nullptr))
        return rc;
    p->t16 = small_tile(u32 * (b ? 2 : 1), 1);
    p->chain = false;
    p->C = a->n_sources == 2 ? a->src_width[1] : 0;
#ifndef ELO_DENSE_F32
    {
        const int C = p->C;
        const auto aligned16 = [](const elo_mlp_args *j) {
            return ((uintptr_t)j->src[0] | (uintptr_t)j->src[1] | (uintptr_t)j->before | (uintptr_t)j->after | (uintptr_t)j->out |
                    (uintptr_t)j->out2) % 16 == 0;
        };
        const bool aligned = aligned16(a) && (!b || aligned16(b));
        p->chain = a->n_sources == 2 && a->src_width[0] == 64 &&
                   (C == 16 || C == 32 || C == 64) && a->n_layers == 2 && a->layers[0].N == 128 && a->layers[1].N == 64 && a->n_layers2 == 2 &&
                   a->layers2[0].N == 128 && a->layers2[1].N == 64 && a->w_before == C && a->w_after == 64 && aligned &&
                   mlp_chain_regime(a->rows, b != nullptr, a->batch_hint, p->mode);
    }
#endif
    p->sv_tiles = 0;
    p->sv_lds = 0;
    const int final_n = a->n_layers2 > 0 ? a->layers2[a->n_layers2 - 1].N : a->layers[a->n_layers - 1].N;
    if (!p->chain && final_n == 64 && a->sv_npoints > 0 && a->rows > 0 && a->rows % a->sv_npoints == 0) {
        const bool t16 = small_tile((a->rows / a->sv_npoints) * (((long)a->sv_npoints + 31) / 32), 1);
        const int tile = t16 ? 16 : 32, groups = b ? 2 : 1;
        const long tiles = ((long)a->sv_npoints + tile - 1) / tile;
        const size_t lds = sizeof(float) * ((size_t)groups * tile * p->S + (b ? 0 : (size_t)tile * 64));
        if (tiles <= ELO_SV_MAX_PARTS && lds <= 64 * 1024) {
            p->sv_tiles = (int)tiles;
            p->sv_lds = lds;
            p->t16 = t16;
        }
    }
    return ELO_OK;
}

extern "C" int elo_mlp_sv_parts(const elo_mlp_args *a, const elo_mlp_args *b)
{
    MlpPlan p;
    if (plan_mlp(a, b, &p, "elo_mlp_sv_parts")) return 0;
    return p.sv_tiles;
}

extern "C" int elo_mlp_fused2(const elo_mlp_args *a, const elo_mlp_args *b, elo_stream_t stream)
{
    const char *who = "elo_mlp_fused";
    MlpPlan plan;
    if (int rc = plan_mlp(a, b, &plan, who)) return rc;
    if (a->rows == 0)
        return a->clear_scratch || a->sv_scratch ? fail(ELO_ERR_ARG, "%s: a clear_* / sv_* side job needs rows to ride on", who) : ELO_OK;
    const int S = plan.S, mode = plan.mode;
    const bool t16 = plan.t16;
    const long u32 = (a->rows + 31) / 32, u16 = (a->rows + 15) / 16;
    JobPair<elo_mlp_args> pair;
    pair.job[0] = *a;
    pair.job[1] = b ? *b : *a;
    if (a->sv_scratch) {
        if (!plan.sv_tiles)
            return fail(ELO_ERR_ARG, "%s: sv_scratch is set but this launch cannot compute softmax_valid's partial sums "
                                     "(elo_mlp_sv_parts returns 0: chain-kernel regime, final width != 64, rows %% sv_npoints != 0 or too many tiles)", who);
        if (!a->sv_xyz) return fail(ELO_ERR_ARG, "%s: sv_scratch without sv_xyz", who);
        if ((b != nullptr) == (a->sv_feature != nullptr))
            return fail(ELO_ERR_ARG, "%s: a paired launch takes its features from job b (sv_feature NULL), a single launch from sv_feature", who);
        if (!b && ((uintptr_t)a->sv_feature & 15)) return fail(ELO_ERR_ARG, "%s: unaligned sv_feature", who);
        const size_t lds = plan.sv_lds;
        const dim3 grid((unsigned)(a->rows / a->sv_npoints) * (unsigned)plan.sv_tiles);
        hipStream_t s = (hipStream_t)stream;
#define CALL_SV(T_, M_)                                                                                                         \
        do {                                                                                                                    \
            if (b) hipLaunchKernelGGL((mlp_sv_kernel<T_, M_, true>), grid, dim3(2 * FUSED_BLOCK), lds, s, pair, S, plan.sv_tiles); \
            else hipLaunchKernelGGL((mlp_sv_kernel<T_, M_, false>), grid, dim3(FUSED_BLOCK), lds, s, pair, S, plan.sv_tiles);     \
        } while (0)
#define CALL_SV_T(M_, t16_) do { if (t16_) CALL_SV(16, M_); else CALL_SV(32, M_); } while (0)
        ELO_PICK_MODE(mode, CALL_SV_T, t16);
#undef CALL_SV_T
#undef CALL_SV
        ++g_sv_ride_launches;
        return check_launch(who);
    }
    const size_t lds = tile_lds_bytes(t16 ? 16 : 32, S);
#ifndef ELO_DENSE_F32
    if (plan.chain) {
        const dim3 rgrid((unsigned)((a->rows + RR_ROWS - 1) / RR_ROWS), b ? 2u : 1u);
        const bool f16 = a->feat_dtype == ELO_F16;
#define CALL(k) ELO_LAUNCH_RR(k, rgrid, (hipStream_t)stream, pair)
        ELO_PICK_RR_C(mlp2_rr_kernel, plan.C, f16, mode, CALL);
#undef CALL
        ++g_rr_launches[3];
        return check_launch(who);
    }
#endif
    const dim3 grid((unsigned)(t16 ? u16 : u32), b ? 2u : 1u);
    hipStream_t s = (hipStream_t)stream;
#define CALL(k) hipLaunchKernelGGL(k, grid, dim3(FUSED_BLOCK), lds, s, pair, S)
    ELO_PICK(mlp_kernel, t16, mode, CALL);
#undef CALL
    return check_launch(who);
}

extern "C" int elo_mlp_fused(const elo_mlp_args *a, elo_stream_t stream) { return elo_mlp_fused2(a, nullptr, stream); }

static int check_cv_features(const char *who, int C, int f16, std::initializer_list<const void *> tensors)
{
    const int per = f16 ? 8 : 4;
    if (C % per != 0) return fail(ELO_ERR_LIMIT, "%s: C = %d must be a multiple of %d (%s feature storage)", who, C, per, f16 ? "fp16" : "fp32");
    if (32 * (C / per) > SEG_ITEMS * FUSED_BLOCK) return fail(ELO_ERR_LIMIT, "%s: C = %d too wide for the tile gather", who, C);
    for (const void *p : tensors)
        if ((uintptr_t)p & 15) return fail(ELO_ERR_ARG, "%s: feature tensors must be 16-byte aligned", who);
    return ELO_OK;
}

static int plan_cv1(const elo_cv1_args *a, TilePlan *p, const char *who)
{
    ELO_REQUIRE(a, who, "null argument block");
    ELO_REQUIRE(a->batch >= 0 && a->npoints > 0 && a->K > 0 && a->H2 > 0 && a->W2 > 0 && a->C > 0, who, "bad sizes");
    if (a->K > 32) return fail(ELO_ERR_LIMIT, "%s: K = %d exceeds the 32-row tile", who, a->K);
    ELO_REQUIRE(a->xyz1 && a->feat1 && a->xyz2 && a->feat2 && a->out, who, "null tensor pointer");
    ELO_REQUIRE(a->group.random_hw || (a->idx && a->mask), who, "neither idx/mask nor a grouping spec");
    ELO_REQUIRE(!a->group.random_hw || a->npoints == a->H2 * a->W2, who, "in-kernel grouping needs npoints == H2*W2");
    if (int rc = check_dtype(a->feat_dtype, who)) return rc;
    if (int rc = check_cv_features(who, a->C, a->feat_dtype == ELO_F16, {a->feat1, a->feat2})) return rc;
    const int CT = 10 + 2 * a->C;
    if (int rc = check_dense(a->cv0, CT, 128, who, "CV_0")) return rc;
    if (int rc = check_dense(a->cv1, 128, 64, who, "CV_1")) return rc;
    if (int rc = check_dense(a->cv2, 64, 64, who, "CV_2")) return rc;
    if (int rc = check_dense(a->cv_xyz, 10, 64, who, "CV_xyz")) return rc;
    if (int rc = check_dense(a->sum_cv0, 128, 128, who, "sum_CV_0")) return rc;
    if (int rc = check_dense(a->sum_cv1, 128, 64, who, "sum_CV_1")) return rc;
    if (int rc = check_points(a->batch, a->npoints, who)) return rc;
    const int cols = 128 + cv1_feat_cols(a->C);
    p->S = row_stride(cols > 192 ? cols : 192);
    if (int rc = products_mode(who, &p->mode, a->cv0, a->cv1, a->cv2, a->cv_xyz, a->sum_cv0, a->sum_cv1)) return rc;
    plan_tiles(p, (long)a->batch * a->npoints, a->K);
    const int KT = a->group.random_hw ? a->group.kernel_h * a->group.kernel_w : 0;
    p->lds = tile_lds_bytes(p->t16 ? 16 : 32, p->S);
    if (sizeof(float) * (((size_t)KT + 3) / 4 * 4 + (size_t)FUSED_WAVES * select_scratch_words(KT, a->K)) > sizeof(float) * (p->t16 ? 16 : 32) * p->S)
        return fail(ELO_ERR_LIMIT, "%s: window %dx%d does not fit the tile for in-kernel grouping", who, a->group.kernel_h, a->group.kernel_w);
    return check_group(a->group, a->H2, a->W2, p->lds, who);
}

extern "C" int elo_cv_stage1_fused(const elo_cv1_args *a, elo_stream_t stream)
{
    const char *who = "elo_cv_stage1_fused";
    TilePlan plan;
    if (int rc = plan_cv1(a, &plan, who)) return rc;
    if ((long)a->batch * a->npoints == 0) return ELO_OK;
#ifndef ELO_DENSE_F32
    if (!a->group.random_hw && cv_chain(a->C, plan.mode)) {
        const int P = RR_ROWS / a->K;
        const dim3 grid((unsigned)(((long)a->batch * a->npoints + P - 1) / P));
        hipStream_t s = (hipStream_t)stream;
        const bool f16 = a->feat_dtype == ELO_F16;
        static_assert(RR_LDS_BYTES <= 64 * 1024, "dynamic LDS within the default limit");
// ... 218 lines not shown
```

efficientlo-net_amd/fused.py:

```python
import ctypes
import os

import torch

from . import _lib as L
from . import tf_util, tuning
from .fused_conv import grouping_entry


def fp32_mfma():
    return bool(L.lib().elo_dense_f32())


PRODUCTS_SPLIT, PRODUCTS_HALF = 0, 1
_products = PRODUCTS_SPLIT


def products_mode():
    return _products


class products:

    def __init__(self, mode):
# ... 223 lines not shown
    L.call2("elo_setconv_fused2", ja[0], jb[0], ja[1])
    return (ja[1], ja[2]), (jb[1], jb[2])


def _mlp_args(sources, layers):
    L.require_gpu(*sources)
    batch_hint = sources[0].shape[0] if sources[0].dim() >= 3 else 0
    srcs, dt, code = _features(*sources)
    srcs = [s.reshape(-1, s.shape[-1]) for s in srcs]
    rows = srcs[0].shape[0]
    out = torch.empty((rows, layers[-1].N), dtype=dt, device=srcs[0].device)
    a = L.MlpArgs()
    a.rows, a.n_sources, a.n_layers, a.layers, a.out = rows, len(srcs), len(layers), _chain(layers), out.data_ptr()
    a.feat_dtype, a.batch_hint = code, batch_hint
    for i, s in enumerate(srcs):
        a.src[i], a.src_width[i] = s.data_ptr(), s.shape[1]
    return a, out, (srcs, layers)


def _ride_clear(a, clear, dt):
    if clear is None:
        return
    if clear.out_feat is not None and clear.out_feat.dtype != dt:
        raise TypeError("the projection buffers and the MLP's features must share one storage dtype")
    B, _N, H, W, C = clear.shape
    a.clear_scratch, a.clear_xyz = clear.scratch.data_ptr(), clear.out_xyz.data_ptr()
    a.clear_feat = clear.out_feat.data_ptr() if clear.out_feat is not None else None
    a.clear_cells, a.clear_C, a.clear_images = B * H * W, C, B
    clear.cleared = True


def _ride_sv(a, b, sv, dt):
    if sv is None:
        return False
    B, N, _ = sv.xyz.shape
    if a.rows != B * N:
        raise ValueError("the SvPartials cloud (%d x %d points) does not match the MLP's %d rows" % (B, N, a.rows))
    a.sv_npoints = N
    parts = L.lib().elo_mlp_sv_parts(ctypes.byref(a), ctypes.byref(b) if b is not None else None)
    if parts <= 0:
        a.sv_npoints = 0
        return False
    a.sv_scratch, a.sv_xyz = sv.scratch.data_ptr(), sv.xyz.data_ptr()
    if b is None:
        feat = sv.feature
        if feat is None or feat.shape != (B, N, 64) or feat.dtype != dt:
            raise ValueError("a single launch takes its (B, N, 64) features of the MLP's storage dtype from SvPartials.feature")
        sv.feature = feat = feat.contiguous()
        a.sv_feature = feat.data_ptr()
    sv.parts = parts
    return True


def mlp(sources, layers, clear=None, sv=None):
    a, out, _keep = _mlp_args(sources, layers)
    if _ride_sv(a, None, sv, out.dtype) or sv is None:
        _ride_clear(a, clear, out.dtype)
    L.call("elo_mlp_fused", a, out)
    return out.reshape(sources[0].shape[:-1] + (layers[-1].N,))


def mlp_pair(sources_a, layers_a, sources_b, layers_b, clear=None, sv=None):
    a, out_a, _ka = _mlp_args(sources_a, layers_a)
    b, out_b, _kb = _mlp_args(sources_b, layers_b)
    if _ride_sv(a, b, sv, out_a.dtype) or sv is None:
        _ride_clear(a, clear, out_a.dtype)
    L.call2("elo_mlp_fused2", a, b, out_a)
    lead = sources_a[0].shape[:-1]
    return out_a.reshape(lead + (layers_a[-1].N,)), out_b.reshape(lead + (layers_b[-1].N,))


def _mlp2_args(sources, layers, before, after, layers2):
    a, out, keep = _mlp_args(sources, layers)
    rows = out.shape[0]
    before, after = _features(before, after, out)[0][:2]
    flat = lambda t: None if t is None else t.reshape(rows, t.shape[-1])
    before, after = flat(before), flat(after)
    out2 = torch.empty((rows, layers2[-1].N), dtype=out.dtype, device=out.device)
    a.n_layers2, a.layers2, a.out2 = len(layers2), _chain(layers2), out2.data_ptr()
    a.before, a.w_before = (before.data_ptr(), before.shape[1]) if before is not None else (None, 0)
    a.after, a.w_after = (after.data_ptr(), after.shape[1]) if after is not None else (None, 0)
    return a, out, out2, (keep, before, after, layers2)


def mlp2_pair(job_a, job_b, clear=None, sv=None):
    a, out_a, out2_a, _ka = _mlp2_args(**job_a)
    b, out_b, out2_b, _kb = _mlp2_args(**job_b)
    if _ride_sv(a, b, sv, out_a.dtype) or sv is None:
        _ride_clear(a, clear, out_a.dtype)
    L.call2("elo_mlp_fused2", a, b, out_a)
    lead = job_a["sources"][0].shape[:-1]
    shape = lambda t: t.reshape(lead + (t.shape[-1],))
    return (shape(out_a), shape(out2_a)), (shape(out_b), shape(out2_b))


THROUGHPUT_BATCH = 4


def _prepass_rows(stage=1, batch=1):
    e = tuning.get("cv_prepass")
    if e is None:
        return 8192 if batch >= THROUGHPUT_BATCH else (20000 if stage == 1 else 65536)
    return (1 << 60) if e == 0 else 0 if e == 1 else int(e)


_HW = {}


def _all_pixels(B, H, W, device):
    key = (B, H, W, str(device))
    hit = _HW.get(key)
    if hit is None:
        hh = torch.arange(H, dtype=torch.int32, device=device).view(1, H, 1, 1).expand(B, H, W, 1)
        ww = torch.arange(W, dtype=torch.int32, device=device).view(1, 1, W, 1).expand(B, H, W, 1)
        hit = torch.cat([hh, ww], -1).reshape(B, H * W, 2).contiguous()
        if hit.is_cuda and torch.cuda.is_current_stream_capturing():
            return hit
        if len(_HW) >= 64:
            _HW.clear()
        _HW[key] = hit
    return hit




def group_prepass(kind, xyz1_grid, xyz2_grid, group, K):
    B, H, W, _ = xyz1_grid.shape
    _, H2, W2, _ = xyz2_grid.shape
    N, kH, kW = H * W, group.kernel_h, group.kernel_w
    idx = torch.empty((B, N, K, 3), dtype=torch.int32, device=xyz1_grid.device)
    mask = torch.empty((B, N, K), dtype=torch.float32, device=xyz1_grid.device)
    large = kind != "select" or -(-W // 64) * H * B >= tuning.get("select_dense_tiles")
    entry = grouping_entry(kind, kH, kW, K, 0, group.stride_h, group.stride_w, large)
    dense = entry.endswith("_dense")
    hw = None if dense else _all_pixels(B, H, W, xyz1_grid.device)
    a = L.GroupArgs(B, H, W, H2, W2, N, kH, kW, K, 0, group.distance, group.stride_h, group.stride_w,
                    xyz1_grid.data_ptr(), xyz2_grid.data_ptr(), None if dense else hw.data_ptr(), group.random_hw.data_ptr(),
                    idx.data_ptr(), None, None, mask.data_ptr())
    L.call(entry, a, idx)
    return idx, mask


def _rr_path(group, B, N, K, C, stage=1):
# ... 111 lines not shown
```

efficientlo-net_amd/model.py:

```python
import time

import torch

from . import _ops, fused, model_util, perm, pwclo_model, tf_util, tuning


def graph_capture(graph):
    import torch.distributed as dist
    if dist.is_available() and dist.is_initialized():
        return torch.cuda.graph(graph, capture_error_mode="thread_local")
    return torch.cuda.graph(graph)


def distinct_queue_streams(device, want, candidates=16, cycles=500_000):
    dev = torch.device(device)
    spin = getattr(torch.cuda, "_sleep", None)
    pool = [torch.cuda.Stream(device=dev) for _ in range(max(candidates, want))]
    if spin is None or want <= 1:
        return pool[:want]

    def timed(streams):
        best = float("inf")
        for _ in range(2):
            torch.cuda.synchronize(dev)
# ... 56 lines not shown
        from . import _lib
        prev = _lib.range_check(True)
        try:
            _lib.range_violations(xyz_f1_proj)
            self.forward(xyz_f1_proj, xyz_f2_proj)
            return _lib.range_violations(xyz_f1_proj)
        finally:
            _lib.range_check(bool(prev))

    def capture(self, batch_size, H_input, W_input, warmup=3, lanes=1, num_points=None, point_stride=3, pose_ring=0, sample=None,
                fresh_orders=0, check_every=0):
        dev = self.device
        if sample is not None:
            bad = self.check_range(sample[:batch_size], sample[batch_size:])
            if bad:
                raise RuntimeError("%d matrix-core operands of this forward lie at or beyond the fp16 range (|x| >= 65504): the "
                                   "fused kernels' hi/lo split would saturate them -- rescale the inputs / weights or run the "
                                   "fp32-MFMA build (ELO_DENSE_F32=1)" % bad)
        side = torch.cuda.Stream(device=dev)
        side.wait_stream(torch.cuda.current_stream(dev))
        def zeros():
            return torch.zeros((2 * batch_size, H_input, W_input, 3), device=dev)
        with torch.cuda.stream(side):
            probe = zeros()
            for _ in range(warmup):
                self.forward(probe[:batch_size], probe[batch_size:])
        torch.cuda.current_stream(dev).wait_stream(side)
        torch.cuda.synchronize(dev)
        self._lanes = []
        if fresh_orders:
            self.perms.enable_pool(int(fresh_orders), lanes, dev)
        streams = distinct_queue_streams(dev, lanes)
        if num_points is not None:
            with torch.cuda.stream(side):
                model_util.input_stage(torch.zeros((batch_size, 2 * num_points, point_stride), device=dev), None, None,
                                       H_input, W_input)
            torch.cuda.synchronize(dev)
        for i in range(lanes):
            both = zeros()
            lane = {"stream": streams[i % len(streams)], "pair": both, "in": (both[:batch_size], both[batch_size:]),
                    "graph": torch.cuda.CUDAGraph(), "replays": 0,
                    "pose": _ops.PoseRing(pose_ring, batch_size, dev) if pose_ring else torch.zeros((batch_size, 7), device=dev)}
            lane["order"] = torch.cuda.Event()
            with torch.cuda.stream(side):
                lane["order"].record()
            if num_points is not None:
                lane["cloud"] = torch.zeros((batch_size, 2 * num_points, point_stride), device=dev)
            if fresh_orders:
                self.perms.active_lane, self.perms.tail_armed = i, False
                with torch.cuda.stream(side):
                    self.forward(both[:batch_size], both[batch_size:])
                torch.cuda.synchronize(dev)
            self.perms.tail_armed = bool(fresh_orders)
            with graph_capture(lane["graph"]):
                if num_points is not None:
                    _pts, staged = model_util.input_stage(lane["cloud"], None, None, H_input, W_input)
                    lane["out"] = self.forward(staged[:batch_size], staged[batch_size:], pose_out=lane["pose"])
                else:
                    lane["out"] = self.forward(*lane["in"], pose_out=lane["pose"])
            if check_every:
                from . import _lib
                lane["graph_checked"], lane["check_every"] = torch.cuda.CUDAGraph(), int(check_every)
                lane["range_counter"] = torch.zeros((1,), dtype=torch.int64, device=dev)
                prev = _lib.range_check(True)
                prev_counter = _lib.set_range_counter(lane["range_counter"].data_ptr())
                try:
                    self.perms.tail_armed = False
                    with torch.cuda.stream(side):
                        self.forward(*lane["in"])
                    torch.cuda.synchronize(dev)
                    self.perms.tail_armed = bool(fresh_orders)
                    with graph_capture(lane["graph_checked"]):
                        if num_points is not None:
                            _pts, staged = model_util.input_stage(lane["cloud"], None, None, H_input, W_input)
                            lane["out_checked"] = self.forward(staged[:batch_size], staged[batch_size:], pose_out=lane["pose"])
                        else:
                            lane["out_checked"] = self.forward(*lane["in"], pose_out=lane["pose"])
                finally:
                    _lib.range_check(bool(prev))
                    _lib.set_range_counter(prev_counter)
                lane["range_counter"].zero_()
            lane["keep"] = _cached_tensors()
            lane["native"] = self._native_submit(lane, dev)
            self._lanes.append(lane)
        self.perms.active_lane, self.perms.tail_armed = 0, False
        torch.cuda.synchronize(dev)
        self._graph, self._static_in, self._static_out = (self._lanes[0]["graph"], self._lanes[0]["in"],
                                                          self._lanes[0]["out"])
        self._captured_at = (self.store.generation, self.perms.generation, tuning.digest())
        self._tuning_seen = tuning.version()
        self.captured_tuning = tuning.snapshot()
        return self

    @staticmethod
    def _native_submit(lane, dev):
        if not tuning.get("native_submit"):
            return None
        from . import _lib
        try:
            execs = [lane[k].raw_cuda_graph_exec() if k in lane else None for k in ("graph", "graph_checked")]
        except (AttributeError, RuntimeError):
            return None
        import ctypes
        pair = lane["pair"]
        return {"submit": _lib.lib().elo_graph_submit, "exec": ctypes.c_void_p(execs[0]), "exec_checked": ctypes.c_void_p(execs[1] or execs[0]),
                "stream": ctypes.c_void_p(lane["stream"].cuda_stream), "dst": ctypes.c_void_p(pair.data_ptr()),
                "nbytes": pair.numel() * pair.element_size(), "event": ctypes.c_void_p(lane["order"].cuda_event), "device": int(dev.index)}

    def _check_fresh(self):
        if self._graph is None:
            raise RuntimeError("no captured graph: call capture() first")
        if self._captured_at[:2] != (self.store.generation, self.perms.generation):
            raise RuntimeError("the captured graph is stale: the variables or the visiting orders changed after capture() "
                               "(checkpoint load, training step or reshuffle) -- call capture() again")
        if self._tuning_seen != tuning.version():
            if self._captured_at[2] == tuning.digest():
                self._tuning_seen = tuning.version()
                return
            raise RuntimeError("the captured graph is stale: the tuning changed after capture() (a graph keeps the kernel forms of "
                               "its capture: tuning.py / elo_set_tuning) -- call capture() again; captured under "
                               "%s, now %s" % (self.captured_tuning, tuning.snapshot()))

    def load_inputs(self, xyz_f1_proj, xyz_f2_proj):
        self._static_in[0].copy_(xyz_f1_proj, non_blocking=True)
        self._static_in[1].copy_(xyz_f2_proj, non_blocking=True)

    def replay(self):
        self._check_fresh()
        return self._replay_lane(self._lanes[0])

    def _replay_lane(self, lane):
        n = lane.get("check_every", 0)
        lane["total"] = lane.get("total", 0) + 1
        checked = n and lane["total"] % n == 0
# ... 136 lines not shown
```

efficientlo-net_amd/pwclo_model.py:

```python
import math
import os

import numpy as np
import torch

from . import _ops, fused, tf_util, tuning
from .model_util import (PreProcess, ProjectPC2SphericalRing, input_stage, preprocess_gt, get_selected_idx, inv_q, mul_point_q, mul_q_point,
                         softmax_valid, warp_and_project)
from .pointnet_util import (cost_volume, down_conv, down_conv_job, flow_predictor, fused_pairs_available, merge_branches,
                            up_conv, up_conv_predict_finish, up_conv_stage1_jobs, up_conv_stage2_jobs)

Down_conv_dis = [0.5, 3.0, 6.0, 12.0]
Up_conv_dis = [3.0, 6.0, 9.0]
Cost_volume_dis = [1.0, 2.0, 4.0]
stride_h_list = [1, 1, 4, 2, 2, 1]
stride_w_list = [1, 1, 8, 2, 2, 2]


def pyramid_sizes(H_input, W_input):
    out_h = [math.ceil(H_input / stride_h_list[0])]
    out_w = [math.ceil(W_input / stride_w_list[0])]
    for i in range(1, 6):
        out_h.append(math.ceil(out_h[i - 1] / stride_h_list[i]))
        out_w.append(math.ceil(out_w[i - 1] / stride_w_list[i]))
# ... 184 lines not shown
            xyz_s = [two(x) for x in xyz_proj]
            xyz_proj_f1, xyz_proj_f2 = [a for a, _ in xyz_s], [b for _, b in xyz_s]
        elif both is not None:
            sel2 = [get_selected_idx(both, stride_h_list[i], stride_w_list[i], out_h_list[i], out_w_list[i])
                    for i in (2, 3, 4, 5)]
            pts, pts_proj, xyz_proj = feature_pyramid(both, zero_features(both), sel2)
            B = batch_size
            half = lambda t, lo, hi: None if t is None else t[lo:hi]
            pts_f1, pts_f2 = [half(p, 0, B) for p in pts], [half(p, B, 2 * B) for p in pts]
            pts_proj_f1 = [half(p, 0, B) for p in pts_proj]
            pts_proj_f2 = [half(p, B, 2 * B) for p in pts_proj]
            xyz_proj_f1, xyz_proj_f2 = [half(x, 0, B) for x in xyz_proj], [half(x, B, 2 * B) for x in xyz_proj]
        else:
            sel1 = [l0_selected_idx, l1_selected_idx, l2_selected_idx, l3_selected_idx]
            points_input_proj = zero_features(xyz_f1_input_proj)
            pts_f1, pts_proj_f1, xyz_proj_f1 = feature_pyramid(xyz_f1_input_proj, points_input_proj, sel1)
            scope.reuse_variables()
            pts_f2, pts_proj_f2, xyz_proj_f2 = feature_pyramid(xyz_f2_input_proj, points_input_proj, sel1)

    l2_points_f1_new = cost_volume(xyz_proj_f1[2], xyz_proj_f2[2], pts_proj_f1[2], pts_proj_f2[2],
                                   kernel_size1=[3, 5], kernel_size2=[5, 35], nsample=4, nsample_q=32,
                                   distance=Cost_volume_dis[2], mlp1=[128, 64, 64], mlp2=[128, 64],
                                   is_training=is_training, bn_decay=bn_decay, scope='flow_embedding_l2_origin',
                                   bn=True, pooling='max', knn=True, corr_func='concat',
                                   side_jobs=[job for job, _ in deferred] or None)
    if deferred:
        l2_points_f1_new, side = l2_points_f1_new
        for f, ((_job, finish), (out, new_xyz)) in enumerate(zip(deferred, side)):
            l3_points, l3_xyz_proj = finish(out, new_xyz)
            if len(deferred) == 1 and l3_points.shape[0] == 2 * batch_size:
                pts_f1[3], pts_f2[3] = l3_points[:batch_size], l3_points[batch_size:]
                xyz_proj_f1[3], xyz_proj_f2[3] = l3_xyz_proj[:batch_size], l3_xyz_proj[batch_size:]
            else:
                (pts_f1 if f == 0 else pts_f2)[3] = l3_points
                (xyz_proj_f1 if f == 0 else xyz_proj_f2)[3] = l3_xyz_proj
    l2_points_new_proj_f1 = l2_points_f1_new.reshape(batch_size, out_h_list[4], out_w_list[4], -1)
    l3_points_f1_cost_volume, _ = down_conv(xyz_proj_f1[2], l2_points_new_proj_f1, l3_selected_idx, K_sample=16,
                                            kernel_size=[5, 9], distance=Down_conv_dis[3], mlp=[128, 64, 64], mlp2=None,
                                            flag_add=False, is_training=is_training, bn_decay=bn_decay,
                                            scope='new_layer3')

    l3_points_predict = l3_points_f1_cost_volume
    l3_points_predict_proj = l3_points_predict.reshape(batch_size, out_h_list[5], out_w_list[5], -1)
    l3_xyz_f1 = xyz_proj_f1[3].reshape(batch_size, -1, 3)
    inference = not is_training

    def projection_buffers(level, g):
        if not inference:
            return None
        return _ops.ProjectionBuffers(batch_size, xyz_proj_f1[level].shape[1] * xyz_proj_f1[level].shape[2],
                                      out_h_list[g], out_w_list[g], pts_f1[level].shape[-1], dev, pts_f1[level].dtype)
    def sv_ride(xyz_bn3, feature=None):
        if inference and fused_pairs_available(is_training) and tuning.get("sv_ride"):
            return _ops.SvPartials(xyz_bn3, feature)
        return None
    def next_warp(level):
        return (xyz_proj_f1[level].reshape(batch_size, -1, 3), pts_f1[level]) if inference else None
    next_buffers = projection_buffers(2, 4)
    sv3 = sv_ride(l3_xyz_f1, l3_points_predict)
    l3_cost_volume_w = flow_predictor(pts_f1[3], None, l3_points_predict, mlp=[128, 64], is_training=is_training,
                                      bn_decay=bn_decay, scope='l3_costvolume_predict_ww',
                                      clear=next_buffers if sv3 is not None else None,
                                      **({"sv": sv3} if sv3 is not None else {}))
    l3_cost_volume_w_proj = l3_cost_volume_w.reshape(batch_size, out_h_list[5], out_w_list[5], -1)
    l3_q, l3_t, l3_q_norm = _estimate_pose(l3_points_predict, l3_cost_volume_w, l3_xyz_f1, 3, None, None,
                                           is_training, clear=next_buffers, warp=next_warp(2), partials=sv3)

    cv_kernel2 = {2: [5, 15], 1: [7, 25], 0: [11, 41]}
    poses = {3: (l3_q_norm, l3_t)}
    q_prev, t_prev = l3_q, l3_t
    coarse_w_proj, coarse_predict_proj, coarse_xyz_proj = l3_cost_volume_w_proj, l3_points_predict_proj, xyz_proj_f1[3]
    for level, g in ((2, 4), (1, 3), (0, 2)):
        q_coarse = q_prev.reshape(batch_size, 1, -1)
        t_coarse = t_prev.reshape(batch_size, 1, -1)
        xyz_f1 = xyz_proj_f1[level].reshape(batch_size, -1, 3)
        _warped, xyz_warp_proj_f1, points_warp_proj_f1 = warp_and_project(
            xyz_f1, pts_f1[level], q_coarse, t_coarse, out_h_list[g], out_w_list[g], next_buffers)
        if PROJECTION_TAP is not None and next_buffers is not None:
            PROJECTION_TAP.append((level, next_buffers.scratch, batch_size, xyz_f1.shape[1], out_h_list[g], out_w_list[g], xyz_warp_proj_f1, _warped))
        next_buffers = projection_buffers(level - 1, g - 1) if level > 0 else None
        xyz_warp_f1 = xyz_warp_proj_f1.reshape(batch_size, -1, 3)
        points_warp_f1 = points_warp_proj_f1.reshape(batch_size, out_h_list[g] * out_w_list[g], -1)

        def branch_cost(side_jobs=None, side_chain=False, upconv=None):
            return cost_volume(xyz_warp_proj_f1, xyz_proj_f2[level], points_warp_proj_f1, pts_proj_f2[level],
                               kernel_size1=[3, 5], kernel_size2=cv_kernel2[level], nsample=4, nsample_q=6,
                               distance=Cost_volume_dis[level], mlp1=[128, 64, 64], mlp2=[128, 64],
                               is_training=is_training, bn_decay=bn_decay, scope='flow_embedding_l%d' % level,
                               bn=True, pooling='max', knn=True, corr_func='concat', side_jobs=side_jobs,
                               **({"side_chain": True} if side_chain else {}),
                               **({"upconv": upconv} if upconv is not None else {}))

        def branch_up(kind, coarse_feat_proj):
            return up_conv(xyz_warp_proj_f1, coarse_xyz_proj, points_warp_proj_f1, coarse_feat_proj,
                           kernel_size=[7, 15], stride_h=stride_h_list[g + 1], stride_w=stride_w_list[g + 1],
                           nsample=8, distance=Up_conv_dis[level], mlp=[128, 64], mlp2=[128, 64],
                           scope='up_sa_layer_layer_l%d%s' % (level, kind), is_training=is_training,
                           bn_decay=bn_decay, knn=True)

        if fused_pairs_available(is_training):
            up = dict(xyz1_proj=xyz_warp_proj_f1, xyz2_proj=coarse_xyz_proj, feat1_proj=points_warp_proj_f1,
                      kernel_size=[7, 15], stride_h=stride_h_list[g + 1], stride_w=stride_w_list[g + 1], nsample=8,
                      distance=Up_conv_dis[level], mlp=[128, 64], mlp2=[128, 64])
            up_w = dict(up, feat2_proj=coarse_w_proj, scope='up_sa_layer_layer_l%dw' % level)
            up_c = dict(up, feat2_proj=coarse_predict_proj, scope='up_sa_layer_layer_l%dcostvolume' % level)
            jobs = up_conv_stage1_jobs(up_w, up_c)
            fp = dict(points_f1=points_warp_f1, mlp=[128, 64])
# ... 72 lines not shown
```

efficientlo-net_amd/tuning.py:

```python
import contextlib
import hashlib
import json
import os

def _prepass(spec):
    return None if spec in (None, "") else int(spec)


_HOST = {
    "fused": ("ELO_FUSED", lambda v: v != "0", True),
    "cv_prepass": ("ELO_CV_PREPASS", _prepass, None),
    "select_dense_tiles": ("ELO_SELECT_DENSE_TILES", int, 1024),
    "merge_points": ("ELO_MERGE_POINTS", int, 8192),
    "merge_level_points": ("ELO_MERGE_LEVEL_POINTS", int, 2000),
    "chain_pair": ("ELO_CHAIN_PAIR", lambda v: v != "0", True),
    "native_submit": ("ELO_NATIVE_SUBMIT", lambda v: v != "0", True),
    "sv_ride": ("ELO_SV_RIDE", lambda v: v != "0", True),
    "upconv_ride": ("ELO_UPCONV_RIDE", lambda v: v != "0", True),
    "train_kernels": ("ELO_TRAIN_KERNELS", lambda v: v != "0", True),
    "train_dense": ("ELO_TRAIN_DENSE", lambda v: v != "0", True),
    "train_dense_rows": ("ELO_TRAIN_DENSE_ROWS", int, 25000),
    "train_siamese_batch": ("ELO_TRAIN_SIAMESE_BATCH", lambda v: v != "0", True),
    "train_dense_fused_dz": ("ELO_TRAIN_DENSE_FUSED_DZ", lambda v: v != "0", True),
    "train_dense_dx_rows": ("ELO_TRAIN_DENSE_DX_ROWS", int, 100000),
}
_LIB = {
    "chain_forms": ("ELO_CV1_RR", 1), "narrow_mfma": ("ELO_SETCONV_NARROW_MFMA", 1), "range_check": ("ELO_RANGE_CHECK", 0),
    "select_dense_waves": ("ELO_SELECT_DENSE_WAVES", 0), "random_dense_rows": ("ELO_DENSE_ROWS", 0),
    "setconv_chain_rows": ("ELO_SETCONV_RR_ROWS", -1), "mlp_chain_rows": ("ELO_MLP_RR_ROWS", -1), "small_tile_units": ("ELO_SMALL_TILE_UNITS", 64),
    "pool_wave": ("ELO_POOL_WAVE", 1),
}


_LIB_BOOLEAN = ("chain_forms", "narrow_mfma", "range_check", "pool_wave")


def _host_from_env():
    out = {}
    for name, (var, parse, default) in _HOST.items():
        raw = os.environ.get(var)
        out[name] = default if raw is None else parse(raw)
    return out


def lib_from_env():
    out = {}
    for name, (var, _default) in _LIB.items():
        raw = os.environ.get(var)
        if raw is not None:
            value = int(raw)
            out[name] = (1 if value else 0) if name in _LIB_BOOLEAN else value
    return out


_host = _host_from_env()
_version = 0


def version():
    return _version


def bump():
    global _version
    _version += 1


def get(name):
    return _host[name]


# ... 46 lines not shown
```

include/elo.h:

```cpp
#ifndef ELO_H_
#define ELO_H_

#ifdef __cplusplus
extern "C" {
#endif

typedef void *elo_stream_t;

typedef enum elo_status {
    ELO_OK = 0,
    ELO_ERR_ARG = -1,
    ELO_ERR_LIMIT = -2,
    ELO_ERR_LAUNCH = -3
} elo_status;

int elo_abi_version(void);
int elo_dense_f32(void);
const char *elo_last_error(void);
int elo_range_check(int enable);
int elo_range_violations(unsigned long long *count, elo_stream_t stream);

int elo_graph_submit(void *graph_exec, elo_stream_t stream, void *dst, const void *src, unsigned long bytes,
                     elo_stream_t producer, void *order_event, int device);

// ... 96 lines not shown
    const void *values;
    int values_stride;
    const float *mask;
    void *out;
    int dtype;
} elo_softmax_pool_args;
int elo_masked_softmax_pool(const elo_softmax_pool_args *a, elo_stream_t stream);

typedef struct elo_perm_refresh_args {
    const int *pool;
    int versions, total;
    int *cursor;
    int *flat, *decoded;
    const int *entry_of;
    const int *table;
    int n_entries;
} elo_perm_refresh_args;
int elo_perm_refresh(const elo_perm_refresh_args *a, elo_stream_t stream);

#define ELO_SV_MAX_PARTS 512
typedef struct elo_softmax_valid_args {
    int batch, npoints, C;
    const float *feature;
    const float *weight;
    const float *xyz;
    float *out;
    float *scratch;
    float *stats;
} elo_softmax_valid_args;
int elo_softmax_valid(const elo_softmax_valid_args *a, elo_stream_t stream);

typedef struct elo_pose_head_args {
    int batch, npoints, C, hidden;
    const void *feature, *weight;
    const float *xyz;
    const float *W_big, *b_big;
    const float *W_q, *b_q;
    const float *W_t, *b_t;
    const float *q_coarse;
    const float *t_coarse;
    float *q, *t, *q_norm;
    float *scratch;
    float *pose7;
    unsigned *clear_scratch;
    float *clear_xyz;
    void *clear_feat;
    long clear_cells;
    int clear_C;
    int feat_dtype;
    int pose7_slots;
    unsigned *pose7_cursor;
    elo_perm_refresh_args next_orders;
    int ready_parts;
} elo_pose_head_args;
int elo_pose_head(const elo_pose_head_args *a, elo_stream_t stream);

typedef struct elo_warp_project_args {
    int batch, npoints, C;
    int H, W;
    float az_res, vert_res, vert_off;
    const float *xyz;
    const void *feat;
    const float *q;
    const float *t;
    float *warped;
    float *out_xyz;
    void *out_feat;
    unsigned *scratch;
    int prepared;
    int feat_dtype;
} elo_warp_project_args;
int elo_warp_project(const elo_warp_project_args *a, elo_stream_t stream);

typedef struct elo_input_stage_args {
    int batch, npoints;
    int point_stride;
    int H, W;
    float az_res, vert_res, vert_off;
    float crop_xy;
    const float *cloud;
    const float *T_trans;
    const int *aug_frame;
    float *points;
    float *out_xyz;
    unsigned *scratch;
} elo_input_stage_args;
int elo_input_stage(const elo_input_stage_args *a, elo_stream_t stream);

typedef struct elo_preprocess_gt_args {
    int batch;
    const float *T_gt;
    const float *T_trans;
    const float *T_trans_inv;
    const int *aug_frame;
    float *q_gt;
    float *t_gt;
} elo_preprocess_gt_args;
int elo_preprocess_gt(const elo_preprocess_gt_args *a, elo_stream_t stream);

int elo_pose_head_warp(const elo_pose_head_args *a, const elo_warp_project_args *w, elo_stream_t stream);

typedef struct elo_group_concat_bwd_args {
    int batch, npoints, K;
    int H2, W2, C;
    const float *grad_out;
    const int *idx;
// ... 208 lines not shown
    int H, W;
    int H2, W2, C;
    const float *xyz1_grid;
    const int *centre_hw;
    const float *centre_xyz;
    const float *src_xyz;
    const void *src_feat;
    const int *idx;
    const float *mask;
    int n_layers;
    elo_dense layers[ELO_MAX_CHAIN];
    void *out;
    float *new_xyz;
    elo_group_spec group;
    int feat_dtype;
    unsigned long long *range_counter;
} elo_setconv_args;
int elo_setconv_fused(const elo_setconv_args *a, elo_stream_t stream);
int elo_setconv_fused2(const elo_setconv_args *a, const elo_setconv_args *b, elo_stream_t stream);

typedef struct elo_mlp_args {
    long rows;
    int n_sources;
    const void *src[3];
    int src_width[3];
    int n_layers;
    elo_dense layers[ELO_MAX_CHAIN];
    void *out;
    int n_layers2;
    elo_dense layers2[ELO_MAX_CHAIN];
    const void *before;
    int w_before;
    const void *after;
    int w_after;
    void *out2;
    int feat_dtype;
    unsigned *clear_scratch;
    float *clear_xyz;
    void *clear_feat;
    long clear_cells;
    int clear_C;
    int clear_images;
    int batch_hint;
    float *sv_scratch;
    const float *sv_xyz;
    const void *sv_feature;
    int sv_npoints;
    unsigned long long *range_counter;
} elo_mlp_args;
#define ELO_THROUGHPUT_BATCH 4
int elo_mlp_fused(const elo_mlp_args *a, elo_stream_t stream);
int elo_mlp_fused2(const elo_mlp_args *a, const elo_mlp_args *b, elo_stream_t stream);
int elo_mlp_sv_parts(const elo_mlp_args *a, const elo_mlp_args *b);

typedef struct elo_cv1_args {
    int batch, npoints, K;
    int H2, W2, C;
    const float *xyz1;
    const void *feat1;
    const float *xyz2;
    const void *feat2;
    const int *idx;
    const float *mask;
    elo_dense cv0, cv1, cv2, cv_xyz, sum_cv0, sum_cv1;
    void *out;
    elo_group_spec group;
    int feat_dtype;
    unsigned long long *range_counter;
} elo_cv1_args;
int elo_cv_stage1_fused(const elo_cv1_args *a, elo_stream_t stream);
int elo_debug_cv1_rr(int on);
int elo_debug_rr_rows(long setconv_rows, long mlp_rows);
int elo_debug_rr_launches(unsigned long long *counts4, int reset);
int elo_debug_sv_ride_launches(unsigned long long *count, int reset);
int elo_debug_chain_pair_launches(unsigned long long *count, int reset);
int elo_debug_upconv_ride_launches(unsigned long long *count, int reset);
int elo_debug_narrow_mfma(int on);
int elo_debug_narrow_launches(unsigned long long *counts2, int reset);
int elo_cv_stage1_setconv_fused(const elo_cv1_args *a, const elo_setconv_args *ja, const elo_setconv_args *jb, elo_stream_t stream);
int elo_cv_stage1_setconv_chain_form(const elo_cv1_args *a, const elo_setconv_args *ja, const elo_setconv_args *jb);
int elo_cv_stage1_setconv_chain(const elo_cv1_args *a, const elo_setconv_args *ja, const elo_setconv_args *jb, elo_stream_t stream);

typedef struct elo_cv2_args {
    int batch, npoints, K;
    int H, W, C;
    const float *xyz1;
    const void *feat1;
    const void *cost;
    const int *idx;
    const float *mask;
    elo_dense xyz_enc, sum_cost0, sum_cost1;
    void *out;
    elo_group_spec group;
    int feat_dtype;
    unsigned long long *range_counter;
} elo_cv2_args;
int elo_cv_stage2_fused(const elo_cv2_args *a, elo_stream_t stream);
int elo_cv_stage2_upconv_form(const elo_cv2_args *a, const elo_mlp_args *ja, const elo_mlp_args *jb);
int elo_cv_stage2_upconv_fused(const elo_cv2_args *a, const elo_mlp_args *ja, const elo_mlp_args *jb, elo_stream_t stream);

#ifdef __cplusplus
}
#endif
#endif
```

Before: 12540.

## Fuse pose head into preceding MLP launch via last-block arrival counter

The MLP launch that produces softmax-valid partials is deferred and then issued together with the pose head (and optional warp projection) as a single kernel. The last tile block to arrive for each batch, tracked by a per-batch atomic arrival word, runs the pose-head body. This removes one kernel launch and the gap between the MLP and the pose head inside the captured graph. In exchange it adds a threadfence and atomic at the end of every tile, and the pose work is serialised onto a single block per batch at the tail of the MLP grid.

```diff
diff --git a/efficientlo-net_amd/_lib.py b/efficientlo-net_amd/_lib.py
--- a/efficientlo-net_amd/_lib.py
+++ b/efficientlo-net_amd/_lib.py
@@ -55,7 +55,7 @@
     ("W_big", _vp), ("b_big", _vp), ("W_q", _vp), ("b_q", _vp), ("W_t", _vp), ("b_t", _vp),
     ("q_coarse", _vp), ("t_coarse", _vp), ("q", _vp), ("t", _vp), ("q_norm", _vp), ("scratch", _vp), ("pose7", _vp),
     ("clear_scratch", _vp), ("clear_xyz", _vp), ("clear_feat", _vp), ("clear_cells", ctypes.c_long), ("clear_C", _i),
-    ("feat_dtype", _i), ("pose7_slots", _i), ("pose7_cursor", _vp), ("next_orders", PermRefreshArgs), ("ready_parts", _i)])
+    ("feat_dtype", _i), ("pose7_slots", _i), ("pose7_cursor", _vp), ("next_orders", PermRefreshArgs), ("ready_parts", _i), ("arrive", _vp)])
 WarpProjectArgs = _struct("elo_warp_project_args", [
     ("batch", _i), ("npoints", _i), ("C", _i), ("H", _i), ("W", _i),
     ("az_res", _f), ("vert_res", _f), ("vert_off", _f),
@@ -202,6 +202,9 @@
     ("elo_setconv_fused2", ctypes.c_int, [ctypes.POINTER(SetconvArgs), ctypes.POINTER(SetconvArgs), _vp]),
     ("elo_mlp_fused2", ctypes.c_int, [ctypes.POINTER(MlpArgs), ctypes.POINTER(MlpArgs), _vp]),
     ("elo_mlp_sv_parts", ctypes.c_int, [ctypes.POINTER(MlpArgs), ctypes.POINTER(MlpArgs)]),
+    ("elo_mlp_pose_ride", ctypes.c_int, [ctypes.POINTER(MlpArgs), ctypes.POINTER(MlpArgs), ctypes.POINTER(PoseHeadArgs), ctypes.POINTER(WarpProjectArgs)]),
+    ("elo_mlp_pose_fused2", ctypes.c_int, [ctypes.POINTER(MlpArgs), ctypes.POINTER(MlpArgs), ctypes.POINTER(PoseHeadArgs), ctypes.POINTER(WarpProjectArgs), _vp]),
+    ("elo_debug_pose_ride_launches", ctypes.c_int, [ctypes.POINTER(ctypes.c_ulonglong), ctypes.c_int]),
     ("elo_cv_stage1_fused", ctypes.c_int, [ctypes.POINTER(Cv1Args), _vp]),
     ("elo_debug_cv1_rr", ctypes.c_int, [ctypes.c_int]),
     ("elo_debug_rr_rows", ctypes.c_int, [ctypes.c_long, ctypes.c_long]),
@@ -316,6 +319,13 @@
         check(getattr(lib(), entry)(ctypes.byref(args_a), ctypes.byref(args_b), stream_ptr(like)))
 
 
+def call_mlp_pose(mlp_a, mlp_b, head, warp, like):
+    _stamp(mlp_a, mlp_b)
+    ref = lambda x: ctypes.byref(x) if x is not None else None
+    with torch.cuda.device(like.device):
+        check(lib().elo_mlp_pose_fused2(ref(mlp_a), ref(mlp_b), ref(head), ref(warp), stream_ptr(like)))
+
+
 def call2n(entry, args_a, args_b, like):
     _stamp(args_a, args_b)
     with torch.cuda.device(like.device):
diff --git a/efficientlo-net_amd/_ops.py b/efficientlo-net_amd/_ops.py
--- a/efficientlo-net_amd/_ops.py
+++ b/efficientlo-net_amd/_ops.py
@@ -369,11 +369,45 @@
 
 class SvPartials:
 
-    def __init__(self, xyz_bn3, feature_bnc=None):
+    def __init__(self, xyz_bn3, feature_bnc=None, hold=False):
         (self.xyz,) = _f32(xyz_bn3)
         self.feature = feature_bnc
         self.scratch = torch.empty((3 * xyz_bn3.shape[0] * L.SV_MAX_PARTS * 64,), dtype=torch.float32, device=xyz_bn3.device)
         self.parts = 0
+        self.hold = hold
+        self.pending = None
+        self.arrive = arrival_words(xyz_bn3.shape[0], xyz_bn3.device)
+
+
+class ArrivalWords:
+
+    def __init__(self, n, device):
+        self.words = torch.zeros((n,), dtype=torch.int32, device=device)
+        self.used = 0
+
+    def take(self, n):
+        if self.used + n > self.words.numel():
+            raise RuntimeError("arrival words exhausted (%d of %d used)" % (self.used, self.words.numel()))
+        self.used += n
+        return self.words[self.used - n:self.used]
+
+
+_arrival_pool = None
+
+
+def set_arrival_pool(pool):
+    global _arrival_pool
+    prev, _arrival_pool = _arrival_pool, pool
+    if pool is not None:
+        pool.used = 0
+    return prev
+
+
+def arrival_words(n, device):
+    pool = _arrival_pool
+    if pool is not None and pool.words.device == device and torch.cuda.is_current_stream_capturing():
+        return pool.take(n)
+    return torch.zeros((n,), dtype=torch.int32, device=device)
 
 
 class PoseRing:
@@ -419,7 +453,11 @@
                                       clear.shape[0] * clear.shape[2] * clear.shape[3], clear.shape[4])
                                      if clear is not None else (None, None, None, 0, 0)), fcode,
                        ring.slots if ring is not None else 0, ring.cursor.data_ptr() if ring is not None else None,
-                       next_orders if next_orders is not None else L.PermRefreshArgs(), ready)
+                       next_orders if next_orders is not None else L.PermRefreshArgs(), ready,
+                       partials.arrive.data_ptr() if partials is not None else None)
+    held = partials.pending if partials is not None else None
+    if held is not None:
+        partials.pending = None
     if ready and clear is not None and not clear.cleared:
         raise ValueError("partials=: the ProjectionBuffers must have been cleared by an earlier launch (fused.mlp(clear=...))")
     if clear is not None and clear.out_feat is not None and clear.out_feat.dtype != fdt:
@@ -440,10 +478,16 @@
         az, vres, voff = projection_constants(Hw, Ww)
         w = L.WarpProjectArgs(Bw, Nw, Cw, Hw, Ww, az, vres, voff, xyz_w.data_ptr(), ptr(feat_w), None, None,
                               warped.data_ptr(), clear.out_xyz.data_ptr(), ptr(clear.out_feat), clear.scratch.data_ptr(), 1, fcode)
-        L.call2("elo_pose_head_warp", a, w, q)
+        if held is not None:
+            L.call_mlp_pose(held[0], held[1], a, w, q)
+        else:
+            L.call2("elo_pose_head_warp", a, w, q)
         clear.result = (warped, clear.out_xyz, clear.out_feat)
         return q, t, q_norm
-    L.call("elo_pose_head", a, q)
+    if held is not None:
+        L.call_mlp_pose(held[0], held[1], a, None, q)
+    else:
+        L.call("elo_pose_head", a, q)
     if clear is not None:
         clear.cleared = True
     return q, t, q_norm
diff --git a/efficientlo-net_amd/csrc/elo_features.hip b/efficientlo-net_amd/csrc/elo_features.hip
--- a/efficientlo-net_amd/csrc/elo_features.hip
+++ b/efficientlo-net_amd/csrc/elo_features.hip
@@ -1,6 +1,7 @@
 #include <type_traits>
 #include "elo_common.h"
 #include "elo_project_device.h"
+#include "elo_pose_device.h"
 
 namespace elo {
 namespace {
@@ -594,16 +595,6 @@
     }
 }
 
-struct SvPartials {
-    float *mx, *den, *acc;
-};
-
-__device__ __forceinline__ SvPartials sv_partials(float *scratch, int batch, int C)
-{
-    const size_t n = (size_t)batch * ELO_SV_MAX_PARTS * C;
-    return SvPartials{scratch, scratch + n, scratch + 2 * n};
-}
-
 template <bool F16>
 __global__ __launch_bounds__(ELO_BLOCK) void softmax_valid_partial_kernel(const void *__restrict__ feature_,
                                                                           const void *__restrict__ weight_,
@@ -674,21 +665,6 @@
     }
 }
 
-__device__ __forceinline__ float sv_merge(const SvPartials &s, int b, int c, int C, int parts)
-{
-    float M = -INFINITY;
-    for (int i = 0; i < parts; ++i) M = fmaxf(M, s.mx[((size_t)b * ELO_SV_MAX_PARTS + i) * C + c]);
-    float D = 0.0f, A = 0.0f;
-    for (int i = 0; i < parts; ++i) {
-        const size_t at = ((size_t)b * ELO_SV_MAX_PARTS + i) * C + c;
-        if (s.den[at] == 0.0f) continue;
-        const float sc = expf(s.mx[at] - M);
-        D += s.den[at] * sc;
-        A += s.acc[at] * sc;
-    }
-    return D > 0.0f ? A / D : 0.0f;
-}
-
 __global__ void softmax_valid_merge_kernel(float *scratch, int batch, int C, int parts, float *out, float *stats)
 {
     const int i = blockIdx.x * blockDim.x + threadIdx.x;
@@ -708,77 +684,9 @@
     }
 }
 
-struct ProjScratch { unsigned *minr, *zflag; int *cell_of; unsigned *rbits; };
-
-__host__ __device__ inline ProjScratch proj_scratch(unsigned *s, size_t cells, size_t images, size_t pts)
-{
-    return ProjScratch{s, s + cells, (int *)(s + cells + ZFLAGS * images), s + cells + ZFLAGS * images + pts};
-}
-
-__device__ __forceinline__ void bin_point(float x, float y, float z, long i, int b, int H, int W, float az_res, float vert_res,
-                                          float vert_off, const ProjScratch &ps)
-{
-    const float r = sqrtf(x * x + y * y + z * z);
-    const float at = atan2f(y, x);
-    const int cell = cell_of_point(at, z, r, H, W, az_res, vert_res, vert_off);
-    const unsigned rb = __float_as_uint(r);
-    ps.cell_of[i] = cell;
-    ps.rbits[i] = rb;
-    if (rb == 0) {
-        const int flag = b * ZFLAGS + zero_kind(at);
-        const unsigned long long zeros = __ballot(1);
-        const int leader = __ffsll((long long)zeros) - 1;
-        if ((int)(threadIdx.x & 63) == leader || flag != __shfl(flag, leader)) ps.zflag[flag] = 0u;
-        return;
-    }
-    unsigned *slot = ps.minr + (long)b * H * W + cell;
-    if (__hip_atomic_load(slot, __ATOMIC_RELAXED, __HIP_MEMORY_SCOPE_AGENT) > rb) atomicMin(slot, rb);
-}
-
-__device__ __forceinline__ void warp_cell_point(const elo_warp_project_args &a, long i, int b, const float *q, const float *t,
-                                                const ProjScratch &ps)
-{
-    float x = a.xyz[i * 3 + 0], y = a.xyz[i * 3 + 1], z = a.xyz[i * 3 + 2];
-    if (q) {
-        const bool keep = !(x == 0.0f && y == 0.0f && z == 0.0f);
-        const float q0 = q[0], q1 = q[1], q2 = q[2], q3 = q[3];
-        const float v0 = q0 * 0.0f - q1 * x - q2 * y - q3 * z;
-        const float v1 = q0 * x + q1 * 0.0f + q2 * z - q3 * y;
-        const float v2 = q0 * y - q1 * z + q2 * 0.0f + q3 * x;
-        const float v3 = q0 * z + q1 * y - q2 * x + q3 * 0.0f;
-        const float n2 = q0 * q0 + q1 * q1 + q2 * q2 + q3 * q3 + 1e-10f;
-        const float i0 = q0 / n2, i1 = -q1 / n2, i2 = -q2 / n2, i3 = -q3 / n2;
-        const float w1 = v0 * i1 + v1 * i0 + v2 * i3 - v3 * i2;
-        const float w2 = v0 * i2 - v1 * i3 + v2 * i0 + v3 * i1;
-        const float w3 = v0 * i3 + v1 * i2 - v2 * i1 + v3 * i0;
-        const float k = keep ? 1.0f : 0.0f;
-        x = (w1 + t[0]) * k; y = (w2 + t[1]) * k; z = (w3 + t[2]) * k;
-        a.warped[i * 3 + 0] = x; a.warped[i * 3 + 1] = y; a.warped[i * 3 + 2] = z;
-    }
-    bin_point(x, y, z, i, b, a.H, a.W, a.az_res, a.vert_res, a.vert_off, ps);
-}
-
-__device__ __forceinline__ void hamilton(const float *a, const float *b, float *r)
-{
-    r[0] = a[0] * b[0] - a[1] * b[1] - a[2] * b[2] - a[3] * b[3];
-    r[1] = a[0] * b[1] + a[1] * b[0] + a[2] * b[3] - a[3] * b[2];
-    r[2] = a[0] * b[2] - a[1] * b[3] + a[2] * b[0] + a[3] * b[1];
-    r[3] = a[0] * b[3] + a[1] * b[2] - a[2] * b[1] + a[3] * b[0];
-}
-
-__device__ __forceinline__ void normalise_q(const float *q, float *o)
-{
-    const float n = sqrtf(q[0] * q[0] + q[1] * q[1] + q[2] * q[2] + q[3] * q[3] + 1e-10f) + 1e-10f;
-    for (int i = 0; i < 4; ++i) o[i] = q[i] / n;
-}
 
 #ifdef ELO_POSE_CLOCK
 __device__ unsigned long long g_pose_clock[4 * 8 + 1];
-#define POSE_STAMP(i) do { if (blockIdx.x == 0 && blockIdx.y == 0 && threadIdx.x == 0) {                                    \
-        if ((i) == 0) pose_slot = (int)(g_pose_clock[32]++ % 4);                                                          \
-        g_pose_clock[pose_slot * 8 + (i)] = __builtin_readcyclecounter(); } } while (0)
-#else
-#define POSE_STAMP(i) do { } while (0)
 #endif
 
 template <int BLOCK>
@@ -786,167 +694,18 @@
                                                           const elo_warp_project_args w, const int with_warp)
 {
     extern __shared__ float sm[];
-    float *feat = sm, *big = sm + a.C, *head = big + a.hidden;
-    const int b = blockIdx.y, tid = threadIdx.x;
-    const SvPartials s = sv_partials(a.scratch, gridDim.y, a.C);
 #ifdef ELO_POSE_CLOCK
     int pose_slot = 0;
+    auto stamp = [&](int i) {
+        if (blockIdx.x == 0 && blockIdx.y == 0 && threadIdx.x == 0) {
+            if (i == 0) pose_slot = (int)(g_pose_clock[32]++ % 4);
+            g_pose_clock[pose_slot * 8 + i] = __builtin_readcyclecounter();
+        }
+    };
+#else
+    auto stamp = [](int) {};
 #endif
-    POSE_STAMP(0);
-    constexpr int HEAD_C = 64;
-    const bool model_head = a.C == HEAD_C && a.hidden == BLOCK;
-    float wb[HEAD_C], wq[4], wt[3], bias_big = 0.0f;
-    auto request_weights = [&]() {
-        const int j = tid;
-#pragma unroll
-        for (int c = 0; c < HEAD_C; ++c) wb[c] = a.W_big[(size_t)c * a.hidden + j];
-#pragma unroll
-        for (int o = 0; o < 4; ++o) wq[o] = a.W_q[(size_t)j * 4 + o];
-#pragma unroll
-        for (int o = 0; o < 3; ++o) wt[o] = a.W_t[(size_t)j * 3 + o];
-        bias_big = a.b_big[j];
-    };
-    float *mpart = head + 8 + 8 * (BLOCK / ELO_WAVE);
-    if (model_head) request_weights();
-    const int c = tid & 63, q = tid >> 6;
-    float M = -INFINITY, D = 0.0f, A = 0.0f;
-    if (c < a.C) {
-        auto trips = [&](auto mine) {
-            constexpr int MINE = decltype(mine)::value;
-            for (int i0 = q; i0 < parts; i0 += 4 * MINE) {
-                float m_[MINE], d_[MINE], a_[MINE];
-#pragma unroll
-                for (int u = 0; u < MINE; ++u) {
-                    const int i = i0 + 4 * u;
-                    const size_t at = ((size_t)b * ELO_SV_MAX_PARTS + (i < parts ? i : 0)) * a.C + c;
-                    m_[u] = s.mx[at]; a_[u] = s.acc[at];
-                    d_[u] = i < parts ? s.den[at] : 0.0f;
-                }
-#pragma unroll
-                for (int u = 0; u < MINE; ++u) {
-                    if (d_[u] == 0.0f) continue;
-                    if (m_[u] > M) { const float sc = exp_acc(M - m_[u]); D = D * sc + d_[u]; A = A * sc + a_[u]; M = m_[u]; }
-                    else { const float sc = exp_acc(m_[u] - M); D += d_[u] * sc; A += a_[u] * sc; }
-                }
-            }
-        };
-        if (parts <= 64) trips(std::integral_constant<int, 16>());
-        else trips(std::integral_constant<int, 32>());
-    }
-    POSE_STAMP(1);
-    mpart[(0 * 4 + q) * 64 + c] = M; mpart[(1 * 4 + q) * 64 + c] = D; mpart[(2 * 4 + q) * 64 + c] = A;
-    __syncthreads();
-    if (tid < 64) {
-        float MM = -INFINITY;
-        for (int i = 0; i < 4; ++i) MM = fmaxf(MM, mpart[(0 * 4 + i) * 64 + tid]);
-        float DD = 0.0f, AA = 0.0f;
-        for (int i = 0; i < 4; ++i) {
-            if (mpart[(1 * 4 + i) * 64 + tid] == 0.0f) continue;
-            const float sc = exp_acc(mpart[(0 * 4 + i) * 64 + tid] - MM);
-            DD += mpart[(1 * 4 + i) * 64 + tid] * sc; AA += mpart[(2 * 4 + i) * 64 + tid] * sc;
-        }
-        if (tid < a.C) feat[tid] = DD > 0.0f ? AA / DD : 0.0f;
-    }
-    for (int c2 = 64 + tid; c2 < a.C; c2 += blockDim.x) feat[c2] = sv_merge(s, b, c2, a.C, parts);
-
-    __syncthreads();
-    POSE_STAMP(2);
-    if (model_head) {
-        float v = bias_big;
-#pragma unroll
-        for (int c = 0; c < HEAD_C; ++c) v += feat[c] * wb[c];
-        big[tid] = v;
-    } else {
-        for (int j = tid; j < a.hidden; j += blockDim.x) {
-            float v = a.b_big[j];
-#pragma unroll 16
-            for (int c = 0; c < a.C; ++c) v += feat[c] * a.W_big[(size_t)c * a.hidden + j];
-            big[j] = v;
-        }
-    }
-    __syncthreads();
-    POSE_STAMP(3);
-    {
-        float part[7] = {0, 0, 0, 0, 0, 0, 0};
-        if (model_head) {
-            const float bj = big[tid];
-#pragma unroll
-            for (int o = 0; o < 4; ++o) part[o] += bj * wq[o];
-#pragma unroll
-            for (int o = 0; o < 3; ++o) part[4 + o] += bj * wt[o];
-        } else {
-            for (int j = tid; j < a.hidden; j += blockDim.x) {
-                const float bj = big[j];
-#pragma unroll
-                for (int o = 0; o < 4; ++o) part[o] += bj * a.W_q[(size_t)j * 4 + o];
-#pragma unroll
-                for (int o = 0; o < 3; ++o) part[4 + o] += bj * a.W_t[(size_t)j * 3 + o];
-            }
-        }
-#pragma unroll
-        for (int o = 0; o < 7; ++o)
-            for (int d = 32; d >= 1; d >>= 1) part[o] += __shfl_xor(part[o], d, ELO_WAVE);
-        float *wsum = head + 8;
-        if ((tid & 63) == 0)
-            for (int o = 0; o < 7; ++o) wsum[(tid >> 6) * 8 + o] = part[o];
-        __syncthreads();
-        if (tid < 7) {
-            float v = tid < 4 ? a.b_q[tid] : a.b_t[tid - 4];
-            for (int w = 0; w < (int)(blockDim.x >> 6); ++w) v += wsum[w * 8 + tid];
-            head[tid] = v;
-        }
-    }
-    __syncthreads();
-    POSE_STAMP(4);
-    if (tid == 0) {
-        float q_det[4], q[4], t[3], qn[4];
-        normalise_q(head, q_det);
-        const float *t_det = head + 4;
-        if (a.q_coarse) {
-            const float *qc = a.q_coarse + b * 4, *tc = a.t_coarse + b * 3;
-            const float tq[4] = {0.0f, tc[0], tc[1], tc[2]};
-            float v[4], w[4], inv[4];
-            hamilton(q_det, tq, v);
-            const float n2 = q_det[0] * q_det[0] + q_det[1] * q_det[1] + q_det[2] * q_det[2] + q_det[3] * q_det[3] + 1e-10f;
-            inv[0] = q_det[0] / n2; inv[1] = -q_det[1] / n2; inv[2] = -q_det[2] / n2; inv[3] = -q_det[3] / n2;
-            hamilton(v, inv, w);
-            hamilton(q_det, qc, q);
-            for (int i = 0; i < 3; ++i) t[i] = w[i + 1] + t_det[i];
-        } else {
-            for (int i = 0; i < 4; ++i) q[i] = q_det[i];
-            for (int i = 0; i < 3; ++i) t[i] = t_det[i];
-        }
-        normalise_q(q, qn);
-        if (blockIdx.x == 0) {
-            for (int i = 0; i < 4; ++i) { a.q[b * 4 + i] = q[i]; a.q_norm[b * 4 + i] = qn[i]; }
-            for (int i = 0; i < 3; ++i) a.t[b * 3 + i] = t[i];
-            if (a.pose7) {
-                float *row = a.pose7 + b * 7;
-                if (a.pose7_slots > 1 && a.pose7_cursor) {
-                    const unsigned at = a.pose7_cursor[b];
-                    a.pose7_cursor[b] = at + 1u;
-                    row += (size_t)(at % (unsigned)a.pose7_slots) * a.batch * 7;
-                }
-                for (int i = 0; i < 4; ++i) row[i] = qn[i];
-                for (int i = 0; i < 3; ++i) row[4 + i] = t[i];
-            }
-        }
-        if (with_warp) {
-            for (int i = 0; i < 4; ++i) head[8 + i] = q[i];
-            for (int i = 0; i < 3; ++i) head[12 + i] = t[i];
-        }
-    }
-    POSE_STAMP(5);
-    if (a.next_orders.pool && blockIdx.x == 0 && blockIdx.y == 0) perm_refresh_block(a.next_orders);
-    POSE_STAMP(6);
-    if (!with_warp) return;
-    __syncthreads();
-    const long n = (long)blockIdx.x * blockDim.x + tid;
-    if (n < w.npoints) {
-        warp_cell_point(w, (long)b * w.npoints + n, b, head + 8, head + 12,
-                        proj_scratch(w.scratch, (size_t)w.batch * w.H * w.W, w.batch, (size_t)w.batch * w.npoints));
-    }
-    POSE_STAMP(7);
+    pose_head_body<BLOCK, 32, 0>(a, parts, w, with_warp, sm, (int)blockIdx.y, (int)gridDim.y, (int)blockIdx.x, (int)threadIdx.x, stamp);
 }
 
 __global__ __launch_bounds__(ELO_BLOCK) void project_init_kernel(unsigned *minr, float *out_xyz, unsigned *out_feat,
@@ -1285,7 +1044,7 @@
     return ELO_OK;
 }
 
-static int pose_head_impl(const elo_pose_head_args *a, const elo_warp_project_args *w, elo_stream_t stream, const char *who)
+static int pose_head_check(const elo_pose_head_args *a, const elo_warp_project_args *w, elo_warp_project_args *wv_out, const char *who)
 {
     ELO_REQUIRE(a, who, "null argument block");
     ELO_REQUIRE(a->batch >= 0 && a->npoints > 0 && a->C > 0 && a->hidden > 0, who, "bad sizes");
@@ -1312,7 +1071,27 @@
     }
     ELO_REQUIRE(a->ready_parts >= 0 && a->ready_parts <= ELO_SV_MAX_PARTS, who, "ready_parts is 0..ELO_SV_MAX_PARTS");
     ELO_REQUIRE(!a->ready_parts || a->C == 64, who, "ready_parts: the partial sums of an MLP launch are 64 channels wide");
+    *wv_out = wv;
+    return ELO_OK;
+}
+
+static int pose_head_pass_b(const elo_warp_project_args &wv, elo_stream_t stream, const char *who)
+{
+    const int f16 = wv.feat_dtype == ELO_F16;
+    const size_t cells = (size_t)wv.batch * wv.H * wv.W, pts = (size_t)wv.batch * wv.npoints;
+    const size_t elems = pts * (3 + (f16 ? wv.C / 2 : wv.C));
+    const unsigned gb = (unsigned)((elems + ELO_BLOCK - 1) / ELO_BLOCK);
+    hipLaunchKernelGGL(scatter_min_kernel, dim3(gb > 4096 ? 4096 : gb), dim3(ELO_BLOCK), 0, (hipStream_t)stream, wv,
+                       proj_scratch(wv.scratch, cells, wv.batch, pts));
+    return check_launch(who);
+}
+
+static int pose_head_impl(const elo_pose_head_args *a, const elo_warp_project_args *w, elo_stream_t stream, const char *who)
+{
+    elo_warp_project_args wv{};
+    if (int rc = pose_head_check(a, w, &wv, who)) return rc;
     if (a->batch == 0) return ELO_OK;
+    const int f16 = a->feat_dtype == ELO_F16;
     hipStream_t s = (hipStream_t)stream;
     {
         const int parts = a->ready_parts ? a->ready_parts : sv_parts(a->npoints);
@@ -1326,23 +1105,53 @@
         else
             hipLaunchKernelGGL(softmax_valid_partial_kernel<false>, pgrid, dim3(ELO_BLOCK), 0, s, a->feature, a->weight, a->xyz,
                                a->npoints, a->C, parts, a->scratch, clear);
-        const size_t lds = sizeof(float) * ((size_t)a->C + a->hidden + 8 + 8 * (ELO_BLOCK / ELO_WAVE) + 3 * 4 * 64);
+        const size_t lds = pose_head_lds(a->C, a->hidden, ELO_BLOCK);
         const unsigned xb = w ? (unsigned)((w->npoints + ELO_BLOCK - 1) / ELO_BLOCK) : 1u;
         hipLaunchKernelGGL((pose_head_kernel<ELO_BLOCK>), dim3(xb, a->batch), dim3(ELO_BLOCK), lds, s, *a, parts, wv, w ? 1 : 0);
     }
-    if (w) {
-        const size_t cells = (size_t)w->batch * w->H * w->W, pts = (size_t)w->batch * w->npoints;
-        const size_t elems = pts * (3 + (f16 ? w->C / 2 : w->C));
-        const unsigned gb = (unsigned)((elems + ELO_BLOCK - 1) / ELO_BLOCK);
-        hipLaunchKernelGGL(scatter_min_kernel, dim3(gb > 4096 ? 4096 : gb), dim3(ELO_BLOCK), 0, s, wv,
-                           proj_scratch(w->scratch, cells, w->batch, pts));
-    }
+    if (w) return pose_head_pass_b(wv, stream, who);
     return check_launch(who);
 }
 
 extern "C" int elo_pose_head(const elo_pose_head_args *a, elo_stream_t stream)
 {
     return pose_head_impl(a, nullptr, stream, "elo_pose_head");
+}
+
+static bool pose_rides(const elo_mlp_args *a, const elo_mlp_args *b, const elo_pose_head_args *p, const elo_warp_project_args *w)
+{
+    size_t lds = 0;
+    if (!p || !mlp_sv_plan(a, b, &lds)) return false;
+    return p->arrive && p->C == 64 && p->hidden == ELO_BLOCK && p->batch == (int)(a->rows / a->sv_npoints) &&
+           (!w || w->npoints <= ELO_BLOCK) && lds >= pose_head_lds(p->C, p->hidden, ELO_BLOCK);
+}
+
+extern "C" int elo_mlp_pose_ride(const elo_mlp_args *a, const elo_mlp_args *b, const elo_pose_head_args *p, const elo_warp_project_args *w)
+{
+    return pose_rides(a, b, p, w) ? 1 : 0;
+}
+
+extern "C" int elo_mlp_pose_fused2(const elo_mlp_args *a, const elo_mlp_args *b, const elo_pose_head_args *p, const elo_warp_project_args *w,
+                                   elo_stream_t stream)
+{
+    const char *who = "elo_mlp_pose_fused";
+    ELO_REQUIRE(a && p, who, "null argument block");
+    ELO_REQUIRE(a->sv_scratch && a->sv_scratch == p->scratch, who, "the pose head merges the partial sums of this launch: p->scratch must be a->sv_scratch");
+    const int parts = elo_mlp_sv_parts(a, b);
+    ELO_REQUIRE(parts > 0, who, "this launch cannot compute softmax_valid's partial sums (elo_mlp_sv_parts returns 0)");
+    elo_pose_head_args head = *p;
+    head.ready_parts = parts;
+    if (!pose_rides(a, b, &head, w)) {
+        if (int rc = mlp_launch(a, b, nullptr, stream, who)) return rc;
+        return pose_head_impl(&head, w, stream, who);
+    }
+    PoseRide ride{};
+    if (int rc = pose_head_check(&head, w, &ride.warp, who)) return rc;
+    ride.head = head;
+    ride.arrive = head.arrive;
+    ride.with_warp = w ? 1 : 0;
+    if (int rc = mlp_launch(a, b, &ride, stream, who)) return rc;
+    return w ? pose_head_pass_b(ride.warp, stream, who) : ELO_OK;
 }
 
 extern "C" int elo_pose_head_warp(const elo_pose_head_args *a, const elo_warp_project_args *w, elo_stream_t stream)
diff --git a/efficientlo-net_amd/csrc/elo_fused.hip b/efficientlo-net_amd/csrc/elo_fused.hip
--- a/efficientlo-net_amd/csrc/elo_fused.hip
+++ b/efficientlo-net_amd/csrc/elo_fused.hip
@@ -1,5 +1,6 @@
 #include "elo_group_device.h"
 #include "elo_project_device.h"
+#include "elo_pose_device.h"
 #include <atomic>
 #include <cstdlib>
 #include <type_traits>
@@ -1105,7 +1106,7 @@
 
 template <int TILE, int MODE, bool PAIR>
 __global__ __launch_bounds__(PAIR ? 2 * FUSED_BLOCK : FUSED_BLOCK, TILE == 32 ? 4 : ELO_TILE_WAVES)
-void mlp_sv_kernel(const JobPair<elo_mlp_args> jobs, const int S, const int tiles_pb)
+void mlp_sv_kernel(const JobPair<elo_mlp_args> jobs, const int S, const int tiles_pb, const PoseRide ride)
 {
     constexpr int C = 64;
     const int group = PAIR ? __builtin_amdgcn_readfirstlane(threadIdx.x >> 8) : 0;
@@ -1153,7 +1154,8 @@
         }
         __syncthreads();
     }
-    if (threadIdx.x >= C) return;
+    if (threadIdx.x >= C && !ride.arrive) return;
+    if (threadIdx.x < C) {
     const unsigned long long okm = __ballot((threadIdx.x < TILE) & (first + vr < end) & !((px == 0.0f) & (py == 0.0f) & (pz == 0.0f)));
     const int c = threadIdx.x;
     const float *logit = lds + c, *value = PAIR ? lds + tile_words + c : staged + c;
@@ -1186,6 +1188,8 @@
     const size_t n = (size_t)(gridDim.x / (unsigned)tiles_pb) * ELO_SV_MAX_PARTS * C;
     const size_t at = ((size_t)b * ELO_SV_MAX_PARTS + t) * C + c;
     sc[at] = M; sc[n + at] = D; sc[2 * n + at] = A;
+    }
+    if (ride.arrive) pose_ride_epilogue<FUSED_BLOCK, TILE == 32 ? 32 : 16, TILE == 32 ? 64 : 32>(ride, lds, b, tiles_pb, (int)(gridDim.x / (unsigned)tiles_pb));
 }
 
 __host__ __device__ __forceinline__ int cv1_feat_cols(int C)
@@ -2656,6 +2660,13 @@
     if (reset) g_upconv_ride_launches.store(0);
     return ELO_OK;
 }
+static std::atomic<unsigned long long> g_pose_ride_launches;
+extern "C" int elo_debug_pose_ride_launches(unsigned long long *count, int reset)
+{
+    if (count) *count = g_pose_ride_launches.load();
+    if (reset) g_pose_ride_launches.store(0);
+    return ELO_OK;
+}
 static std::atomic<unsigned long long> g_sv_ride_launches;
 extern "C" int elo_debug_sv_ride_launches(unsigned long long *count, int reset)
 {
@@ -2896,9 +2907,8 @@
     return p.sv_tiles;
 }
 
-extern "C" int elo_mlp_fused2(const elo_mlp_args *a, const elo_mlp_args *b, elo_stream_t stream)
-{
-    const char *who = "elo_mlp_fused";
+int elo::mlp_launch(const elo_mlp_args *a, const elo_mlp_args *b, const PoseRide *ride, elo_stream_t stream, const char *who)
+{
     MlpPlan plan;
     if (int rc = plan_mlp(a, b, &plan, who)) return rc;
     if (a->rows == 0)
@@ -2920,18 +2930,21 @@
         const size_t lds = plan.sv_lds;
         const dim3 grid((unsigned)(a->rows / a->sv_npoints) * (unsigned)plan.sv_tiles);
         hipStream_t s = (hipStream_t)stream;
+        const PoseRide rv = ride ? *ride : PoseRide{};
 #define CALL_SV(T_, M_)                                                                                                         \
         do {                                                                                                                    \
-            if (b) hipLaunchKernelGGL((mlp_sv_kernel<T_, M_, true>), grid, dim3(2 * FUSED_BLOCK), lds, s, pair, S, plan.sv_tiles); \
-            else hipLaunchKernelGGL((mlp_sv_kernel<T_, M_, false>), grid, dim3(FUSED_BLOCK), lds, s, pair, S, plan.sv_tiles);     \
+            if (b) hipLaunchKernelGGL((mlp_sv_kernel<T_, M_, true>), grid, dim3(2 * FUSED_BLOCK), lds, s, pair, S, plan.sv_tiles, rv); \
+            else hipLaunchKernelGGL((mlp_sv_kernel<T_, M_, false>), grid, dim3(FUSED_BLOCK), lds, s, pair, S, plan.sv_tiles, rv);     \
         } while (0)
 #define CALL_SV_T(M_, t16_) do { if (t16_) CALL_SV(16, M_); else CALL_SV(32, M_); } while (0)
         ELO_PICK_MODE(mode, CALL_SV_T, t16);
 #undef CALL_SV_T
 #undef CALL_SV
         ++g_sv_ride_launches;
+        if (ride) ++g_pose_ride_launches;
         return check_launch(who);
     }
+    if (ride) return fail(ELO_ERR_ARG, "%s: a pose head can only ride on a launch that computes its partial sums (sv_scratch)", who);
     const size_t lds = tile_lds_bytes(t16 ? 16 : 32, S);
 #ifndef ELO_DENSE_F32
     if (plan.chain) {
@@ -2952,7 +2965,17 @@
     return check_launch(who);
 }
 
+extern "C" int elo_mlp_fused2(const elo_mlp_args *a, const elo_mlp_args *b, elo_stream_t stream) { return mlp_launch(a, b, nullptr, stream, "elo_mlp_fused"); }
+
 extern "C" int elo_mlp_fused(const elo_mlp_args *a, elo_stream_t stream) { return elo_mlp_fused2(a, nullptr, stream); }
+
+int elo::mlp_sv_plan(const elo_mlp_args *a, const elo_mlp_args *b, size_t *lds)
+{
+    MlpPlan plan;
+    if (!a || plan_mlp(a, b, &plan, "elo_mlp_pose_ride") || a->rows == 0) return 0;
+    *lds = plan.sv_lds;
+    return plan.sv_tiles;
+}
 
 static int check_cv_features(const char *who, int C, int f16, std::initializer_list<const void *> tensors)
 {
diff --git a/efficientlo-net_amd/csrc/elo_pose_device.h b/efficientlo-net_amd/csrc/elo_pose_device.h
--- /dev/null
+++ b/efficientlo-net_amd/csrc/elo_pose_device.h
@@ -0,0 +1,299 @@
+#pragma once
+#include <type_traits>
+#include "elo_common.h"
+#include "elo_project_device.h"
+
+namespace elo {
+
+struct PoseRide { elo_pose_head_args head; elo_warp_project_args warp; unsigned *arrive; int with_warp; };
+
+int mlp_launch(const elo_mlp_args *a, const elo_mlp_args *b, const PoseRide *ride, elo_stream_t stream, const char *who);
+int mlp_sv_plan(const elo_mlp_args *a, const elo_mlp_args *b, size_t *lds);
+inline size_t pose_head_lds(int C, int hidden, int block) { return sizeof(float) * ((size_t)C + hidden + 8 + 8 * (block / ELO_WAVE) + 3 * 4 * 64); }
+
+struct SvPartials {
+    float *mx, *den, *acc;
+};
+
+__device__ __forceinline__ SvPartials sv_partials(float *scratch, int batch, int C)
+{
+    const size_t n = (size_t)batch * ELO_SV_MAX_PARTS * C;
+    return SvPartials{scratch, scratch + n, scratch + 2 * n};
+}
+
+__device__ __forceinline__ float sv_merge(const SvPartials &s, int b, int c, int C, int parts)
+{
+    float M = -INFINITY;
+    for (int i = 0; i < parts; ++i) M = fmaxf(M, s.mx[((size_t)b * ELO_SV_MAX_PARTS + i) * C + c]);
+    float D = 0.0f, A = 0.0f;
+    for (int i = 0; i < parts; ++i) {
+        const size_t at = ((size_t)b * ELO_SV_MAX_PARTS + i) * C + c;
+        if (s.den[at] == 0.0f) continue;
+        const float sc = expf(s.mx[at] - M);
+        D += s.den[at] * sc;
+        A += s.acc[at] * sc;
+    }
+    return D > 0.0f ? A / D : 0.0f;
+}
+
+struct ProjScratch { unsigned *minr, *zflag; int *cell_of; unsigned *rbits; };
+
+__host__ __device__ inline ProjScratch proj_scratch(unsigned *s, size_t cells, size_t images, size_t pts)
+{
+    return ProjScratch{s, s + cells, (int *)(s + cells + ZFLAGS * images), s + cells + ZFLAGS * images + pts};
+}
+
+__device__ __forceinline__ void bin_point(float x, float y, float z, long i, int b, int H, int W, float az_res, float vert_res,
+                                          float vert_off, const ProjScratch &ps)
+{
+    const float r = sqrtf(x * x + y * y + z * z);
+    const float at = atan2f(y, x);
+    const int cell = cell_of_point(at, z, r, H, W, az_res, vert_res, vert_off);
+    const unsigned rb = __float_as_uint(r);
+    ps.cell_of[i] = cell;
+    ps.rbits[i] = rb;
+    if (rb == 0) {
+        const int flag = b * ZFLAGS + zero_kind(at);
+        const unsigned long long zeros = __ballot(1);
+        const int leader = __ffsll((long long)zeros) - 1;
+        if ((int)(threadIdx.x & 63) == leader || flag != __shfl(flag, leader)) ps.zflag[flag] = 0u;
+        return;
+    }
+    unsigned *slot = ps.minr + (long)b * H * W + cell;
+    if (__hip_atomic_load(slot, __ATOMIC_RELAXED, __HIP_MEMORY_SCOPE_AGENT) > rb) atomicMin(slot, rb);
+}
+
+__device__ __forceinline__ void warp_cell_point(const elo_warp_project_args &a, long i, int b, const float *q, const float *t,
+                                                const ProjScratch &ps)
+{
+    float x = a.xyz[i * 3 + 0], y = a.xyz[i * 3 + 1], z = a.xyz[i * 3 + 2];
+    if (q) {
+        const bool keep = !(x == 0.0f && y == 0.0f && z == 0.0f);
+        const float q0 = q[0], q1 = q[1], q2 = q[2], q3 = q[3];
+        const float v0 = q0 * 0.0f - q1 * x - q2 * y - q3 * z;
+        const float v1 = q0 * x + q1 * 0.0f + q2 * z - q3 * y;
+        const float v2 = q0 * y - q1 * z + q2 * 0.0f + q3 * x;
+        const float v3 = q0 * z + q1 * y - q2 * x + q3 * 0.0f;
+        const float n2 = q0 * q0 + q1 * q1 + q2 * q2 + q3 * q3 + 1e-10f;
+        const float i0 = q0 / n2, i1 = -q1 / n2, i2 = -q2 / n2, i3 = -q3 / n2;
+        const float w1 = v0 * i1 + v1 * i0 + v2 * i3 - v3 * i2;
+        const float w2 = v0 * i2 - v1 * i3 + v2 * i0 + v3 * i1;
+        const float w3 = v0 * i3 + v1 * i2 - v2 * i1 + v3 * i0;
+        const float k = keep ? 1.0f : 0.0f;
+        x = (w1 + t[0]) * k; y = (w2 + t[1]) * k; z = (w3 + t[2]) * k;
+        a.warped[i * 3 + 0] = x; a.warped[i * 3 + 1] = y; a.warped[i * 3 + 2] = z;
+    }
+    bin_point(x, y, z, i, b, a.H, a.W, a.az_res, a.vert_res, a.vert_off, ps);
+}
+
+__device__ __forceinline__ void hamilton(const float *a, const float *b, float *r)
+{
+    r[0] = a[0] * b[0] - a[1] * b[1] - a[2] * b[2] - a[3] * b[3];
+    r[1] = a[0] * b[1] + a[1] * b[0] + a[2] * b[3] - a[3] * b[2];
+    r[2] = a[0] * b[2] - a[1] * b[3] + a[2] * b[0] + a[3] * b[1];
+    r[3] = a[0] * b[3] + a[1] * b[2] - a[2] * b[1] + a[3] * b[0];
+}
+
+__device__ __forceinline__ void normalise_q(const float *q, float *o)
+{
+    const float n = sqrtf(q[0] * q[0] + q[1] * q[1] + q[2] * q[2] + q[3] * q[3] + 1e-10f) + 1e-10f;
+    for (int i = 0; i < 4; ++i) o[i] = q[i] / n;
+}
+
+template <int BLOCK, int TRIP, int WCHUNK, class Stamp>
+__device__ __forceinline__ void pose_head_body(const elo_pose_head_args &a, const int parts, const elo_warp_project_args &w,
+                                               const int with_warp, float *sm, const int b, const int batch, const int xb,
+                                               const int tid, Stamp stamp)
+{
+    float *feat = sm, *big = sm + a.C, *head = big + a.hidden;
+    const bool on = tid < BLOCK;
+    const SvPartials s = sv_partials(a.scratch, batch, a.C);
+    stamp(0);
+    constexpr int HEAD_C = 64;
+    const bool model_head = a.C == HEAD_C && a.hidden == BLOCK;
+    constexpr bool WHOLE = WCHUNK == 0 || WCHUNK == HEAD_C;
+    float wb[WHOLE ? HEAD_C : 1], wq[4], wt[3], bias_big = 0.0f;
+    auto request_weights = [&]() {
+        const int j = tid;
+        if constexpr (WHOLE) {
+#pragma unroll
+            for (int c = 0; c < HEAD_C; ++c) wb[c] = a.W_big[(size_t)c * a.hidden + j];
+        }
+#pragma unroll
+        for (int o = 0; o < 4; ++o) wq[o] = a.W_q[(size_t)j * 4 + o];
+#pragma unroll
+        for (int o = 0; o < 3; ++o) wt[o] = a.W_t[(size_t)j * 3 + o];
+        bias_big = a.b_big[j];
+    };
+    float *mpart = head + 8 + 8 * (BLOCK / ELO_WAVE);
+    if (WCHUNK == 0 && model_head && on) request_weights();
+    const int c = tid & 63, q = tid >> 6;
+    float M = -INFINITY, D = 0.0f, A = 0.0f;
+    if (on && c < a.C) {
+        auto trips = [&](auto mine) {
+            constexpr int MINE = decltype(mine)::value;
+            for (int i0 = q; i0 < parts; i0 += 4 * MINE) {
+                float m_[MINE], d_[MINE], a_[MINE];
+#pragma unroll
+                for (int u = 0; u < MINE; ++u) {
+                    const int i = i0 + 4 * u;
+                    const size_t at = ((size_t)b * ELO_SV_MAX_PARTS + (i < parts ? i : 0)) * a.C + c;
+                    m_[u] = s.mx[at]; a_[u] = s.acc[at];
+                    d_[u] = i < parts ? s.den[at] : 0.0f;
+                }
+#pragma unroll
+                for (int u = 0; u < MINE; ++u) {
+                    if (d_[u] == 0.0f) continue;
+                    if (m_[u] > M) { const float sc = exp_acc(M - m_[u]); D = D * sc + d_[u]; A = A * sc + a_[u]; M = m_[u]; }
+                    else { const float sc = exp_acc(m_[u] - M); D += d_[u] * sc; A += a_[u] * sc; }
+                }
+            }
+        };
+        if (parts <= 64) trips(std::integral_constant<int, 16>());
+        else trips(std::integral_constant<int, TRIP>());
+    }
+    stamp(1);
+    if (WCHUNK != 0 && model_head && on) request_weights();
+    if (on) { mpart[(0 * 4 + q) * 64 + c] = M; mpart[(1 * 4 + q) * 64 + c] = D; mpart[(2 * 4 + q) * 64 + c] = A; }
+    __syncthreads();
+    if (tid < 64) {
+        float MM = -INFINITY;
+        for (int i = 0; i < 4; ++i) MM = fmaxf(MM, mpart[(0 * 4 + i) * 64 + tid]);
+        float DD = 0.0f, AA = 0.0f;
+        for (int i = 0; i < 4; ++i) {
+            if (mpart[(1 * 4 + i) * 64 + tid] == 0.0f) continue;
+            const float sc = exp_acc(mpart[(0 * 4 + i) * 64 + tid] - MM);
+            DD += mpart[(1 * 4 + i) * 64 + tid] * sc; AA += mpart[(2 * 4 + i) * 64 + tid] * sc;
+        }
+        if (tid < a.C) feat[tid] = DD > 0.0f ? AA / DD : 0.0f;
+    }
+    if (on)
+        for (int c2 = 64 + tid; c2 < a.C; c2 += BLOCK) feat[c2] = sv_merge(s, b, c2, a.C, parts);
+
+    __syncthreads();
+    stamp(2);
+    if (!on) {
+    } else if (model_head) {
+        float v = bias_big;
+        if constexpr (WHOLE) {
+#pragma unroll
+            for (int c = 0; c < HEAD_C; ++c) v += feat[c] * wb[c];
+        } else {
+            for (int c0 = 0; c0 < HEAD_C; c0 += WCHUNK) {
+                float wc[WCHUNK];
+#pragma unroll
+                for (int c = 0; c < WCHUNK; ++c) wc[c] = a.W_big[(size_t)(c0 + c) * a.hidden + tid];
+#pragma unroll
+                for (int c = 0; c < WCHUNK; ++c) v += feat[c0 + c] * wc[c];
+            }
+        }
+        big[tid] = v;
+    } else {
+        for (int j = tid; j < a.hidden; j += BLOCK) {
+            float v = a.b_big[j];
+#pragma unroll 16
+            for (int c = 0; c < a.C; ++c) v += feat[c] * a.W_big[(size_t)c * a.hidden + j];
+            big[j] = v;
+        }
+    }
+    __syncthreads();
+    stamp(3);
+    if (on) {
+        float part[7] = {0, 0, 0, 0, 0, 0, 0};
+        if (model_head) {
+            const float bj = big[tid];
+#pragma unroll
+            for (int o = 0; o < 4; ++o) part[o] += bj * wq[o];
+#pragma unroll
+            for (int o = 0; o < 3; ++o) part[4 + o] += bj * wt[o];
+        } else {
+            for (int j = tid; j < a.hidden; j += BLOCK) {
+                const float bj = big[j];
+#pragma unroll
+                for (int o = 0; o < 4; ++o) part[o] += bj * a.W_q[(size_t)j * 4 + o];
+#pragma unroll
+                for (int o = 0; o < 3; ++o) part[4 + o] += bj * a.W_t[(size_t)j * 3 + o];
+            }
+        }
+#pragma unroll
+        for (int o = 0; o < 7; ++o)
+            for (int d = 32; d >= 1; d >>= 1) part[o] += __shfl_xor(part[o], d, ELO_WAVE);
+        float *wsum = head + 8;
+        if ((tid & 63) == 0)
+            for (int o = 0; o < 7; ++o) wsum[(tid >> 6) * 8 + o] = part[o];
+    }
+    __syncthreads();
+    if (tid < 7) {
+        const float *wsum = head + 8;
+        float v = tid < 4 ? a.b_q[tid] : a.b_t[tid - 4];
+        for (int wv = 0; wv < BLOCK / ELO_WAVE; ++wv) v += wsum[wv * 8 + tid];
+        head[tid] = v;
+    }
+    __syncthreads();
+    stamp(4);
+    if (tid == 0) {
+        float q_det[4], q[4], t[3], qn[4];
+        normalise_q(head, q_det);
+        const float *t_det = head + 4;
+        if (a.q_coarse) {
+            const float *qc = a.q_coarse + b * 4, *tc = a.t_coarse + b * 3;
+            const float tq[4] = {0.0f, tc[0], tc[1], tc[2]};
+            float v[4], w[4], inv[4];
+            hamilton(q_det, tq, v);
+            const float n2 = q_det[0] * q_det[0] + q_det[1] * q_det[1] + q_det[2] * q_det[2] + q_det[3] * q_det[3] + 1e-10f;
+            inv[0] = q_det[0] / n2; inv[1] = -q_det[1] / n2; inv[2] = -q_det[2] / n2; inv[3] = -q_det[3] / n2;
+            hamilton(v, inv, w);
+            hamilton(q_det, qc, q);
+            for (int i = 0; i < 3; ++i) t[i] = w[i + 1] + t_det[i];
+        } else {
+            for (int i = 0; i < 4; ++i) q[i] = q_det[i];
+            for (int i = 0; i < 3; ++i) t[i] = t_det[i];
+        }
+        normalise_q(q, qn);
+        if (xb == 0) {
+            for (int i = 0; i < 4; ++i) { a.q[b * 4 + i] = q[i]; a.q_norm[b * 4 + i] = qn[i]; }
+            for (int i = 0; i < 3; ++i) a.t[b * 3 + i] = t[i];
+            if (a.pose7) {
+                float *row = a.pose7 + b * 7;
+                if (a.pose7_slots > 1 && a.pose7_cursor) {
+                    const unsigned at = a.pose7_cursor[b];
+                    a.pose7_cursor[b] = at + 1u;
+                    row += (size_t)(at % (unsigned)a.pose7_slots) * a.batch * 7;
+                }
+                for (int i = 0; i < 4; ++i) row[i] = qn[i];
+                for (int i = 0; i < 3; ++i) row[4 + i] = t[i];
+            }
+        }
+        if (with_warp) {
+            for (int i = 0; i < 4; ++i) head[8 + i] = q[i];
+            for (int i = 0; i < 3; ++i) head[12 + i] = t[i];
+        }
+    }
+    stamp(5);
+    if (a.next_orders.pool && xb == 0 && b == 0) perm_refresh_block(a.next_orders);
+    stamp(6);
+    if (!with_warp) return;
+    __syncthreads();
+    const long n = (long)xb * BLOCK + tid;
+    if (on && n < w.npoints) {
+        warp_cell_point(w, (long)b * w.npoints + n, b, head + 8, head + 12,
+                        proj_scratch(w.scratch, (size_t)w.batch * w.H * w.W, w.batch, (size_t)w.batch * w.npoints));
+    }
+    stamp(7);
+}
+
+template <int BLOCK, int TRIP, int WCHUNK>
+__device__ __forceinline__ void pose_ride_epilogue(const PoseRide &ride, float *lds, const int b, const int tiles_pb, const int batch)
+{
+    __threadfence();
+    __syncthreads();
+    int *arrived = reinterpret_cast<int *>(lds);
+    if (threadIdx.x == 0) *arrived = (int)atomicAdd(ride.arrive + b, 1u);
+    __syncthreads();
+    if (*arrived != tiles_pb - 1) return;
+    if (threadIdx.x == 0) __hip_atomic_store(ride.arrive + b, 0u, __ATOMIC_RELAXED, __HIP_MEMORY_SCOPE_AGENT);
+    __threadfence();
+    pose_head_body<BLOCK, TRIP, WCHUNK>(ride.head, tiles_pb, ride.warp, ride.with_warp, lds, b, batch, 0, (int)threadIdx.x, [](int) {});
+}
+
+}
diff --git a/efficientlo-net_amd/fused.py b/efficientlo-net_amd/fused.py
--- a/efficientlo-net_amd/fused.py
+++ b/efficientlo-net_amd/fused.py
@@ -299,20 +299,31 @@
     return True
 
 
+def _launch_mlp(a, b, out, sv, rode):
+    if rode and sv.hold:
+        if sv.pending is not None:
+            raise RuntimeError("this SvPartials already holds a launch no pose head has taken")
+        sv.pending = (a, b, out)
+        return
+    L.call2n("elo_mlp_fused2", a, b, out)
+
+
 def mlp(sources, layers, clear=None, sv=None):
     a, out, _keep = _mlp_args(sources, layers)
-    if _ride_sv(a, None, sv, out.dtype) or sv is None:
+    rode = _ride_sv(a, None, sv, out.dtype)
+    if rode or sv is None:
         _ride_clear(a, clear, out.dtype)
-    L.call("elo_mlp_fused", a, out)
+    _launch_mlp(a, None, out, sv, rode)
     return out.reshape(sources[0].shape[:-1] + (layers[-1].N,))
 
 
 def mlp_pair(sources_a, layers_a, sources_b, layers_b, clear=None, sv=None):
     a, out_a, _ka = _mlp_args(sources_a, layers_a)
     b, out_b, _kb = _mlp_args(sources_b, layers_b)
-    if _ride_sv(a, b, sv, out_a.dtype) or sv is None:
+    rode = _ride_sv(a, b, sv, out_a.dtype)
+    if rode or sv is None:
         _ride_clear(a, clear, out_a.dtype)
-    L.call2("elo_mlp_fused2", a, b, out_a)
+    _launch_mlp(a, b, out_a, sv, rode)
     lead = sources_a[0].shape[:-1]
     return out_a.reshape(lead + (layers_a[-1].N,)), out_b.reshape(lead + (layers_b[-1].N,))
 
@@ -333,9 +344,10 @@
 def mlp2_pair(job_a, job_b, clear=None, sv=None):
     a, out_a, out2_a, _ka = _mlp2_args(**job_a)
     b, out_b, out2_b, _kb = _mlp2_args(**job_b)
-    if _ride_sv(a, b, sv, out_a.dtype) or sv is None:
+    rode = _ride_sv(a, b, sv, out_a.dtype)
+    if rode or sv is None:
         _ride_clear(a, clear, out_a.dtype)
-    L.call2("elo_mlp_fused2", a, b, out_a)
+    _launch_mlp(a, b, out_a, sv, rode)
     lead = job_a["sources"][0].shape[:-1]
     shape = lambda t: t.reshape(lead + (t.shape[-1],))
     return (shape(out_a), shape(out2_a)), (shape(out_b), shape(out2_b))
diff --git a/efficientlo-net_amd/model.py b/efficientlo-net_amd/model.py
--- a/efficientlo-net_amd/model.py
+++ b/efficientlo-net_amd/model.py
@@ -132,6 +132,8 @@
                     self.forward(both[:batch_size], both[batch_size:])
                 torch.cuda.synchronize(dev)
             self.perms.tail_armed = bool(fresh_orders)
+            lane["arrive"] = _ops.ArrivalWords(4 * batch_size, dev)
+            _ops.set_arrival_pool(lane["arrive"])
             with graph_capture(lane["graph"]):
                 if num_points is not None:
                     _pts, staged = model_util.input_stage(lane["cloud"], None, None, H_input, W_input)
@@ -150,6 +152,7 @@
                         self.forward(*lane["in"])
                     torch.cuda.synchronize(dev)
                     self.perms.tail_armed = bool(fresh_orders)
+                    _ops.set_arrival_pool(lane["arrive"])
                     with graph_capture(lane["graph_checked"]):
                         if num_points is not None:
                             _pts, staged = model_util.input_stage(lane["cloud"], None, None, H_input, W_input)
@@ -160,6 +163,7 @@
                     _lib.range_check(bool(prev))
                     _lib.set_range_counter(prev_counter)
                 lane["range_counter"].zero_()
+            _ops.set_arrival_pool(None)
             lane["keep"] = _cached_tensors()
             lane["native"] = self._native_submit(lane, dev)
             self._lanes.append(lane)
diff --git a/efficientlo-net_amd/pwclo_model.py b/efficientlo-net_amd/pwclo_model.py
--- a/efficientlo-net_amd/pwclo_model.py
+++ b/efficientlo-net_amd/pwclo_model.py
@@ -260,7 +260,7 @@
                                       out_h_list[g], out_w_list[g], pts_f1[level].shape[-1], dev, pts_f1[level].dtype)
     def sv_ride(xyz_bn3, feature=None):
         if inference and fused_pairs_available(is_training) and tuning.get("sv_ride"):
-            return _ops.SvPartials(xyz_bn3, feature)
+            return _ops.SvPartials(xyz_bn3, feature, hold=tuning.get("pose_ride"))
         return None
     def next_warp(level):
         return (xyz_proj_f1[level].reshape(batch_size, -1, 3), pts_f1[level]) if inference else None
diff --git a/efficientlo-net_amd/tuning.py b/efficientlo-net_amd/tuning.py
--- a/efficientlo-net_amd/tuning.py
+++ b/efficientlo-net_amd/tuning.py
@@ -17,6 +17,7 @@
     "native_submit": ("ELO_NATIVE_SUBMIT", lambda v: v != "0", True),
     "sv_ride": ("ELO_SV_RIDE", lambda v: v != "0", True),
     "upconv_ride": ("ELO_UPCONV_RIDE", lambda v: v != "0", True),
+    "pose_ride": ("ELO_POSE_RIDE", lambda v: v != "0", True),
     "train_kernels": ("ELO_TRAIN_KERNELS", lambda v: v != "0", True),
     "train_dense": ("ELO_TRAIN_DENSE", lambda v: v != "0", True),
     "train_dense_rows": ("ELO_TRAIN_DENSE_ROWS", int, 25000),
diff --git a/include/elo.h b/include/elo.h
--- a/include/elo.h
+++ b/include/elo.h
@@ -172,6 +172,7 @@
     unsigned *pose7_cursor;
     elo_perm_refresh_args next_orders;
     int ready_parts;
+    unsigned *arrive;
 } elo_pose_head_args;
 int elo_pose_head(const elo_pose_head_args *a, elo_stream_t stream);
 
@@ -486,6 +487,9 @@
 int elo_mlp_fused(const elo_mlp_args *a, elo_stream_t stream);
 int elo_mlp_fused2(const elo_mlp_args *a, const elo_mlp_args *b, elo_stream_t stream);
 int elo_mlp_sv_parts(const elo_mlp_args *a, const elo_mlp_args *b);
+int elo_mlp_pose_ride(const elo_mlp_args *a, const elo_mlp_args *b, const elo_pose_head_args *p, const elo_warp_project_args *w);
+int elo_mlp_pose_fused2(const elo_mlp_args *a, const elo_mlp_args *b, const elo_pose_head_args *p, const elo_warp_project_args *w,
+                        elo_stream_t stream);
 
 typedef struct elo_cv1_args {
     int batch, npoints, K;
@@ -509,6 +513,7 @@
 int elo_debug_sv_ride_launches(unsigned long long *count, int reset);
 int elo_debug_chain_pair_launches(unsigned long long *count, int reset);
 int elo_debug_upconv_ride_launches(unsigned long long *count, int reset);
+int elo_debug_pose_ride_launches(unsigned long long *count, int reset);
 int elo_debug_narrow_mfma(int on);
 int elo_debug_narrow_launches(unsigned long long *counts2, int reset);
 int elo_cv_stage1_setconv_fused(const elo_cv1_args *a, const elo_setconv_args *ja, const elo_setconv_args *jb, elo_stream_t stream);
```

New measurement: 9866. 0.787x the previous value.
